# Meowuu7/equi-articulated-pose

Measured on AMD Instinct MI355X. Metric: point-clouds/sec (4096 pts, 60 anchors) fwd+bwd, higher is better.
Workload: dtype f32; 1 GPU; 8 x 4096-pt synthetic laptop clouds per GPU, 3-block inter backbone 1->64->128->512 (NN=64,K=24,A=60), forward+backward+Adam; clouds_per_gpu=8, points=4096, anchors=60

## Files before the change

### equi-articulated-pose_amd/csrc/bn_act.hip

```cpp
#include "common.h"

namespace {

constexpr int TB = 256;
constexpr int VPT = 8;
constexpr int SEG = TB * VPT * 4;

__device__ __forceinline__ float wave_sum(float v) {
#pragma unroll
    for (int o = 32; o > 0; o >>= 1) v += __shfl_xor(v, o);
    return v;
}

__device__ __forceinline__ void block_reduce2(float a, float b, float *pa, float *pb) {
    __shared__ float sa[TB / 64], sb[TB / 64];
    a = wave_sum(a); b = wave_sum(b);
    if ((threadIdx.x & 63) == 0) { sa[threadIdx.x >> 6] = a; sb[threadIdx.x >> 6] = b; }
    __syncthreads();
    if (threadIdx.x == 0) {
        float ta = 0.f, tb = 0.f;
#pragma unroll
        for (int i = 0; i < TB / 64; ++i) { ta += sa[i]; tb += sb[i]; }
        *pa = ta; *pb = tb;
    }
// ... 96 lines not shown
    const size_t o = ((size_t)ci * gridDim.z + bi) * nseg + seg;
    block_reduce2(s, q, pg + o, pgx + o);
}

template <bool CLOUD>
__global__ __launch_bounds__(TB) void bn_act_bwd_apply_kernel(int c, long n, float slope, const float *__restrict__ gy,
                                                             const float *__restrict__ x, const float *__restrict__ scale,
                                                             const float *__restrict__ shift, const float *__restrict__ mean,
                                                             const float *__restrict__ invstd, const float *__restrict__ k2,
                                                             const float *__restrict__ k3, float *__restrict__ gx,
                                                             const float *__restrict__ mask, int na) {
    const int seg = blockIdx.x, ci = blockIdx.y, bi = blockIdx.z;
    const int si = CLOUD ? bi * c + ci : ci;
    const float sc = scale[si], sh = shift[si], mu = mean[si], is = invstd[si], c2 = k2[si], c3 = k3[si];
    const size_t r0 = ((size_t)bi * c + ci) * n;
    const float *mrow = (CLOUD && mask) ? mask + (size_t)bi * (unsigned)(n / na) : nullptr;
    const long base = (long)seg * SEG;
    auto one = [&](float g, float xv, float m) {
        const float pre = fmaf(xv, sc, sh);
        const float gg = pre > 0.f ? g : g * slope;
        if (CLOUD) return fmaf(-m, fmaf((xv - mu) * is, c3, c2), gg * sc);
        return fmaf(gg, sc, -c2) - ((xv - mu) * is) * c3;
    };
#pragma unroll
    for (int v = 0; v < VPT; ++v) {
        const long i = base + ((long)v * TB + threadIdx.x) * 4;
        if (i + 3 < n) {
            const float4 g = *reinterpret_cast<const float4 *>(gy + r0 + i);
            const float4 a = *reinterpret_cast<const float4 *>(x + r0 + i);
            const float m = mrow ? mrow[(unsigned)i / (unsigned)na] : 1.f;
            *reinterpret_cast<float4 *>(gx + r0 + i) = make_float4(one(g.x, a.x, m), one(g.y, a.y, m), one(g.z, a.z, m), one(g.w, a.w, m));
        } else {
            for (long j = i; j < n; ++j) gx[r0 + j] = one(gy[r0 + j], x[r0 + j], mrow ? mrow[(unsigned)j / (unsigned)na] : 1.f);
        }
    }
}

constexpr int RM_PIECES = 16;
__global__ __launch_bounds__(256) void bn_act_bwd_apply_rowmax_kernel(int c, long n4, int nq, float slope, const float4 *__restrict__ gy,
                                                                      const float4 *__restrict__ x, const float *__restrict__ scale,
                                                                      const float *__restrict__ shift, const float *__restrict__ mean,
                                                                      const float *__restrict__ invstd, const float *__restrict__ k2,
                                                                      const float *__restrict__ k3, float4 *__restrict__ gx,
                                                                      unsigned *__restrict__ rowmax) {
    __shared__ unsigned s_max[256][4];
    const int ci = blockIdx.y, bi = blockIdx.z, t = threadIdx.x;
    const int T = nq * (256 / nq);
    const float sc = scale[ci], sh = shift[ci], mu = mean[ci], is = invstd[ci], c2 = k2[ci], c3 = k3[ci];
    const size_t r0 = ((size_t)bi * c + ci) * (size_t)n4;
    const long base = (long)blockIdx.x * RM_PIECES * T;
    auto one = [&](float g, float xv) {
        const float pre = fmaf(xv, sc, sh);
        const float gg = pre > 0.f ? g : g * slope;
        return fmaf(gg, sc, -c2) - ((xv - mu) * is) * c3;
    };
    unsigned m0 = 0, m1 = 0, m2 = 0, m3 = 0;
    if (t < T) {
        float4 g[RM_PIECES], a[RM_PIECES];
#pragma unroll
        for (int v = 0; v < RM_PIECES; ++v) {
            const long i = base + (long)v * T + t;
            if (i < n4) { g[v] = gy[r0 + i]; a[v] = x[r0 + i]; }
        }
#pragma unroll
        for (int v = 0; v < RM_PIECES; ++v) {
            const long i = base + (long)v * T + t;
            if (i < n4) {
                const float4 o = make_float4(one(g[v].x, a[v].x), one(g[v].y, a[v].y), one(g[v].z, a[v].z), one(g[v].w, a[v].w));
                gx[r0 + i] = o;
                m0 = max(m0, __float_as_uint(o.x) & 0x7fffffffu); m1 = max(m1, __float_as_uint(o.y) & 0x7fffffffu);
                m2 = max(m2, __float_as_uint(o.z) & 0x7fffffffu); m3 = max(m3, __float_as_uint(o.w) & 0x7fffffffu);
            }
        }
    }
    s_max[t][0] = m0; s_max[t][1] = m1; s_max[t][2] = m2; s_max[t][3] = m3;
    __syncthreads();
    if (t < 4 * nq) {
        unsigned v = 0;
        for (int u = t >> 2; u < T; u += nq) v = max(v, s_max[u][t & 3]);
        if (v) atomicMax(rowmax + ((size_t)bi * c + ci) * (4 * nq) + t, v);
    }
}

__global__ __launch_bounds__(256) void bn_act_bwd_reduce_fromy_kernel(int c, long n4, int nq, int nblk, float slope, float inv_slope, const float4 *__restrict__ gy,
                                                                      const float4 *__restrict__ y, const float *__restrict__ beta,
                                                                      const float *__restrict__ inv_gamma, float *__restrict__ pg, float *__restrict__ pgx,
                                                                      unsigned *__restrict__ gmax, unsigned *__restrict__ xmax) {
    __shared__ unsigned s_max[256][8];
    const int ci = blockIdx.y, bi = blockIdx.z, t = threadIdx.x;
    const int T = nq * (256 / nq);
    const float be = beta[ci], ig = inv_gamma[ci];
    const size_t r0 = ((size_t)bi * c + ci) * (size_t)n4;
    const long base = (long)blockIdx.x * RM_PIECES * T;
    float s = 0.f, q = 0.f;
    unsigned mg[4] = {0, 0, 0, 0}, mx[4] = {0, 0, 0, 0};
    if (t < T) {
        float4 g[RM_PIECES], a[RM_PIECES];
#pragma unroll
        for (int v = 0; v < RM_PIECES; ++v) {
            const long i = base + (long)v * T + t;
            if (i < n4) { g[v] = gy[r0 + i]; a[v] = y[r0 + i]; }
        }
#pragma unroll
        for (int v = 0; v < RM_PIECES; ++v) {
            const long i = base + (long)v * T + t;
            if (i < n4) {
                const float gv[4] = {g[v].x, g[v].y, g[v].z, g[v].w}, yv[4] = {a[v].x, a[v].y, a[v].z, a[v].w};
#pragma unroll
                for (int e = 0; e < 4; ++e) {
                    const bool pos = yv[e] > 0.f;
                    const float gg = pos ? gv[e] : gv[e] * slope, xh = ((pos ? yv[e] : yv[e] * inv_slope) - be) * ig;
                    s += gg;
                    q = fmaf(gg, xh, q);
                    mg[e] = max(mg[e], __float_as_uint(gg) & 0x7fffffffu);
                    mx[e] = max(mx[e], __float_as_uint(xh) & 0x7fffffffu);
                }
            }
        }
    }
#pragma unroll
    for (int e = 0; e < 4; ++e) { s_max[t][e] = mg[e]; s_max[t][4 + e] = mx[e]; }
    const size_t o = ((size_t)ci * gridDim.z + bi) * nblk + blockIdx.x;
    block_reduce2(s, q, pg + o, pgx + o);
    if (t < 4 * nq) {
        unsigned vg = 0, vx = 0;
        for (int u = t >> 2; u < T; u += nq) { vg = max(vg, s_max[u][t & 3]); vx = max(vx, s_max[u][4 + (t & 3)]); }
        const size_t at = ((size_t)bi * c + ci) * (4 * nq) + t;
        if (vg) atomicMax(gmax + at, vg);
        if (vx) atomicMax(xmax + at, vx);
    }
}

inline int nseg_of(long n) { return (int)((n + SEG - 1) / SEG); }

}

extern "C" int eap_bn_act_segments(int64_t n) { return nseg_of((long)n); }

extern "C" int eap_bn_stats_f32(int b, int c, int64_t n, const float *x, float *psum, float *psq, eap_stream_t stream) {
    if (b <= 0 || c <= 0 || n <= 0) return 0;
    if ((n & 3) != 0) return eap::bad_arg("bn_stats: row length must be a multiple of 4");
    const int nseg = nseg_of(n);
    return eap::run_kernel("bn_stats", bn_stats_kernel<false>, nseg, c, b, dim3(TB), 0, eap::S(stream), c, (long)n, nseg, x, psum, psq, (const float *)nullptr, 1);
}

extern "C" int eap_bn_act_fwd_f32(int b, int c, int64_t n, float slope, const float *x, const float *scale,
                                  const float *shift, float *y, eap_stream_t stream) {
    if (b <= 0 || c <= 0 || n <= 0) return 0;
    if ((n & 3) != 0) return eap::bad_arg("bn_act_fwd: row length must be a multiple of 4");
    return eap::run_kernel("bn_act_fwd", bn_act_fwd_kernel<false, false>, nseg_of(n), c, b, dim3(TB), 0, eap::S(stream), c, (long)n, slope, x, scale, shift,
                           (const float *)nullptr, y);
}

extern "C" int eap_bn_act_add_fwd_f32(int b, int c, int64_t n, float slope, const float *x, const float *scale,
                                      const float *shift, const float *res, float *y, eap_stream_t stream) {
    if (b <= 0 || c <= 0 || n <= 0) return 0;
    if ((n & 3) != 0) return eap::bad_arg("bn_act_add_fwd: row length must be a multiple of 4");
    return eap::run_kernel("bn_act_add_fwd", bn_act_fwd_kernel<true, false>, nseg_of(n), c, b, dim3(TB), 0, eap::S(stream), c, (long)n, slope, x, scale, shift,
                           res, y);
}

extern "C" int eap_bn_act_bwd_reduce_f32(int b, int c, int64_t n, float slope, const float *gy, const float *x,
                                         const float *scale, const float *shift, const float *mean,
                                         const float *invstd, float *pg, float *pgx, eap_stream_t stream) {
    if (b <= 0 || c <= 0 || n <= 0) return 0;
    if ((n & 3) != 0) return eap::bad_arg("bn_act_bwd_reduce: row length must be a multiple of 4");
    const int nseg = nseg_of(n);
    return eap::run_kernel("bn_act_bwd_reduce", bn_act_bwd_reduce_kernel<false>, nseg, c, b, dim3(TB), 0, eap::S(stream), c, (long)n, nseg, slope, gy, x,
                           scale, shift, mean, invstd, pg, pgx);
}

extern "C" int eap_bn_act_bwd_apply_f32(int b, int c, int64_t n, float slope, const float *gy, const float *x,
                                        const float *scale, const float *shift, const float *mean,
                                        const float *invstd, const float *k2, const float *k3, float *gx,
                                        eap_stream_t stream) {
    if (b <= 0 || c <= 0 || n <= 0) return 0;
    if ((n & 3) != 0) return eap::bad_arg("bn_act_bwd_apply: row length must be a multiple of 4");
    return eap::run_kernel("bn_act_bwd_apply", bn_act_bwd_apply_kernel<false>, nseg_of(n), c, b, dim3(TB), 0, eap::S(stream), c, (long)n, slope, gy, x,
                           scale, shift, mean, invstd, k2, k3, gx, (const float *)nullptr, 1);
}

extern "C" int eap_bn_act_bwd_apply_rowmax_f32(int b, int c, int64_t n, int na, float slope, const float *gy, const float *x,
                                               const float *scale, const float *shift, const float *mean,
                                               const float *invstd, const float *k2, const float *k3, float *gx, uint32_t *rowmax,
                                               eap_stream_t stream) {
    if (b <= 0 || c <= 0 || n <= 0) return 0;
    if (na <= 0 || (na & 3) != 0 || na > 256 || n % na != 0 ||
        ((reinterpret_cast<uintptr_t>(gy) | reinterpret_cast<uintptr_t>(x) | reinterpret_cast<uintptr_t>(gx)) & 15) != 0)
        return eap::bad_arg("bn_act_bwd_apply_rowmax: rows of [points][na], na a multiple of 4 up to 256, 16-byte aligned tensors");
    hipStream_t s = eap::S(stream);
    if (int e = eap::hip_fail(hipMemsetAsync(rowmax, 0, sizeof(uint32_t) * (size_t)b * c * na, s), "bn_act_bwd_apply_rowmax memset")) return e;
    const int nq = na / 4, T = nq * (256 / nq);
    const long n4 = (long)(n / 4);
    return eap::run_kernel("bn_act_bwd_apply_rowmax", bn_act_bwd_apply_rowmax_kernel, eap::cdiv(n4, (long)RM_PIECES * T), c, b, dim3(256), 0, s, c, n4, nq,
                           slope, reinterpret_cast<const float4 *>(gy), reinterpret_cast<const float4 *>(x), scale, shift, mean, invstd, k2, k3,
                           reinterpret_cast<float4 *>(gx), rowmax);
}

extern "C" int eap_bn_act_fromy_blocks(int64_t n, int na) {
    if (na <= 0 || (na & 3) != 0 || na > 256) return 0;
    const int nq = na / 4, T = nq * (256 / nq);
    const long n4 = (long)(n / 4);
    return (int)((n4 + (long)RM_PIECES * T - 1) / ((long)RM_PIECES * T));
}

extern "C" int eap_bn_act_bwd_reduce_fromy_f32(int b, int c, int64_t n, int na, float slope, const float *gy, const float *y, const float *beta,
                                               const float *inv_gamma, float *pg, float *pgx, uint32_t *gmax, uint32_t *xmax, eap_stream_t stream) {
    if (b <= 0 || c <= 0 || n <= 0) return 0;
    if (na <= 0 || (na & 3) != 0 || na > 256 || n % na != 0 || !(slope > 0.f) ||
        ((reinterpret_cast<uintptr_t>(gy) | reinterpret_cast<uintptr_t>(y)) & 15) != 0)
        return eap::bad_arg("bn_act_bwd_reduce_fromy: rows of [points][na], na a multiple of 4 up to 256, 16-byte aligned tensors, a positive slope");
    hipStream_t s = eap::S(stream);
    if (int e = eap::hip_fail(hipMemsetAsync(gmax, 0, sizeof(uint32_t) * (size_t)b * c * na, s), "bn_act_bwd_reduce_fromy memset")) return e;
    if (int e = eap::hip_fail(hipMemsetAsync(xmax, 0, sizeof(uint32_t) * (size_t)b * c * na, s), "bn_act_bwd_reduce_fromy memset")) return e;
    const int nq = na / 4, nblk = eap_bn_act_fromy_blocks(n, na);
    return eap::run_kernel("bn_act_bwd_reduce_fromy", bn_act_bwd_reduce_fromy_kernel, nblk, c, b, dim3(256), 0, s, c, (long)(n / 4), nq, nblk, slope,
                           1.0f / slope, reinterpret_cast<const float4 *>(gy), reinterpret_cast<const float4 *>(y), beta, inv_gamma, pg, pgx, gmax, xmax);
}

namespace {
inline int cloud_dims(const char *who, int b, int c, long n, int na, bool masked) {
    char buf[200];
    if ((n & 3) != 0 || n >= (1l << 31)) {
        snprintf(buf, sizeof(buf), "%s: row length must be a multiple of 4 below 2^31", who);
        return eap::bad_arg(buf);
    }
    if (masked && (na <= 0 || (na & 3) != 0 || n % na != 0)) {
        snprintf(buf, sizeof(buf), "%s: with a mask a row is [points][na], na a multiple of 4", who);
        return eap::bad_arg(buf);
    }
    return 0;
}
}

extern "C" int eap_bn_stats_masked_f32(int b, int c, int64_t n, int na, const float *x, const float *mask, float *psum, float *psq,
                                       eap_stream_t stream) {
    if (b <= 0 || c <= 0 || n <= 0) return 0;
    if (!mask) return eap::bad_arg("bn_stats_masked: mask is null");
    if (int e = cloud_dims("bn_stats_masked", b, c, (long)n, na, true)) return e;
    const int nseg = nseg_of(n);
    return eap::run_kernel("bn_stats_masked", bn_stats_kernel<true>, nseg, c, b, dim3(TB), 0, eap::S(stream), c, (long)n, nseg, x, psum, psq, mask, na);
}

extern "C" int eap_bn_act_cloud_fwd_f32(int b, int c, int64_t n, float slope, const float *x, const float *scale, const float *shift,
                                        float *y, eap_stream_t stream) {
    if (b <= 0 || c <= 0 || n <= 0) return 0;
    if (int e = cloud_dims("bn_act_cloud_fwd", b, c, (long)n, 0, false)) return e;
    return eap::run_kernel("bn_act_cloud_fwd", bn_act_fwd_kernel<false, true>, nseg_of(n), c, b, dim3(TB), 0, eap::S(stream), c, (long)n, slope, x, scale,
                           shift, (const float *)nullptr, y);
}

extern "C" int eap_bn_act_cloud_bwd_reduce_f32(int b, int c, int64_t n, float slope, const float *gy, const float *x, const float *scale,
                                               const float *shift, const float *mean, const float *invstd, float *pg, float *pgx,
                                               eap_stream_t stream) {
    if (b <= 0 || c <= 0 || n <= 0) return 0;
    if (int e = cloud_dims("bn_act_cloud_bwd_reduce", b, c, (long)n, 0, false)) return e;
    const int nseg = nseg_of(n);
    return eap::run_kernel("bn_act_cloud_bwd_reduce", bn_act_bwd_reduce_kernel<true>, nseg, c, b, dim3(TB), 0, eap::S(stream), c, (long)n, nseg, slope, gy, x,
                           scale, shift, mean, invstd, pg, pgx);
}

extern "C" int eap_bn_act_cloud_bwd_apply_f32(int b, int c, int64_t n, int na, float slope, const float *gy, const float *x,
                                              const float *scale, const float *shift, const float *mean, const float *invstd,
                                              const float *k2, const float *k3, const float *mask, float *gx, eap_stream_t stream) {
    if (b <= 0 || c <= 0 || n <= 0) return 0;
    if (int e = cloud_dims("bn_act_cloud_bwd_apply", b, c, (long)n, na, mask != nullptr)) return e;
    return eap::run_kernel("bn_act_cloud_bwd_apply", bn_act_bwd_apply_kernel<true>, nseg_of(n), c, b, dim3(TB), 0, eap::S(stream), c, (long)n, slope, gy, x,
                           scale, shift, mean, invstd, k2, k3, gx, mask, mask ? na : 1);
}
```

### equi-articulated-pose_amd/csrc/common.h

```cpp
#pragma once
#include <hip/hip_runtime.h>
#include <stdint.h>
#include <stdio.h>

#include <atomic>

#include "../../include/eap_hip.h"

namespace eap {

void set_error(const char *msg);
void set_kernel(const char *name);

static inline int check_launch(const char *what) {
    hipError_t e = hipGetLastError();
    if (e != hipSuccess) {
        char buf[256];
        snprintf(buf, sizeof(buf), "%s: %s", what, hipGetErrorString(e));
        set_error(buf);
        return (int)e;
    }
    return 0;
}

static inline int bad_arg(const char *what) {
    set_error(what);
    return (int)hipErrorInvalidValue;
}

static inline int hip_fail(hipError_t e, const char *what) {
    if (e == hipSuccess) return 0;
    char buf[256];
    snprintf(buf, sizeof(buf), "%s: %s", what, hipGetErrorString(e));
    set_error(buf);
    return (int)e;
}

static inline hipStream_t S(eap_stream_t s) { return (hipStream_t)s; }

static inline long long cdiv(long long a, long long b) { return (a + b - 1) / b; }

template <typename... P>
static inline bool aligned16(const P *...p) { return ((reinterpret_cast<uintptr_t>(p) | ... | (uintptr_t)0) & 15) == 0; }

static inline int launch_dims(const char *what, long long gx, long long gy, long long gz, dim3 block, dim3 *grid) {
    const bool block_ok = block.x >= 1 && block.y >= 1 && block.z >= 1 && block.x <= 1024 && block.y <= 1024 && block.z <= 1024 &&
                          block.x * block.y * block.z <= 1024;
    if (!block_ok || gx < 1 || gy < 1 || gz < 1 || gx > 0xffffffffLL / block.x || gy > 65535 || gz > 65535) {
        char buf[256];
        snprintf(buf, sizeof(buf), "%s: grid (%lld, %lld, %lld) x block (%u, %u, %u) is outside the launch limits: every size >= 1, block <= 1024 "
                 "threads, grid.x * block.x < 2^32, grid.y and grid.z <= 65535", what, gx, gy, gz, block.x, block.y, block.z);
        return bad_arg(buf);
    }
    *grid = dim3((unsigned)gx, (unsigned)gy, (unsigned)gz);
    return 0;
}

struct LdsOptIn {
    std::atomic<const void *> kernel{nullptr};
    std::atomic<unsigned> bytes[64] = {};
};
inline LdsOptIn g_lds_opt_in[256];

static inline int allow_dynamic_lds(const void *kernel, size_t bytes, const char *what) {
    int dev = 0;
    if (int e = hip_fail(hipGetDevice(&dev), what)) return e;
    std::atomic<unsigned> *seen = nullptr;
    for (size_t i = 0, h = reinterpret_cast<uintptr_t>(kernel) >> 4; i < 256 && dev >= 0 && dev < 64; ++i) {
        LdsOptIn &slot = g_lds_opt_in[(h + i) & 255];
        const void *k = slot.kernel.load(std::memory_order_acquire);
        if (k == nullptr && slot.kernel.compare_exchange_strong(k, kernel, std::memory_order_acq_rel)) k = kernel;
        if (k == kernel) { seen = &slot.bytes[dev]; break; }
    }
    unsigned have = seen ? seen->load(std::memory_order_acquire) : 0u;
    if (have >= bytes) return 0;
    for (;;) {
        if (int e = hip_fail(hipFuncSetAttribute(kernel, hipFuncAttributeMaxDynamicSharedMemorySize, (int)bytes), what)) return e;
        if (!seen || seen->compare_exchange_strong(have, (unsigned)bytes, std::memory_order_acq_rel)) return 0;
        if (have > bytes) bytes = have;
    }
}

template <typename K, typename... Args>
static inline int run_kernel(const char *what, K kernel, long long gx, long long gy, long long gz, dim3 block, size_t lds_bytes, hipStream_t s,
                             Args... args) {
    dim3 grid;
    if (int e = launch_dims(what, gx, gy, gz, block, &grid)) return e;
    if (lds_bytes)
        if (int e = allow_dynamic_lds(reinterpret_cast<const void *>(kernel), lds_bytes, what)) return e;
    hipLaunchKernelGGL(kernel, grid, block, lds_bytes, s, args...);
    return check_launch(what);
}

int side_fork(hipStream_t s, hipStream_t *side);
int side_join(hipStream_t s);
struct SideJoin {
    hipStream_t s;
    bool armed = true;
    explicit SideJoin(hipStream_t stream) : s(stream) {}
    ~SideJoin() { if (armed) side_join(s); }
    int join() { armed = false; return side_join(s); }
};

int reduce_slabs(const float *ws, float *C, long long mn, int N, int slabs, long long ldc, hipStream_t s, const char *what);
bool group_lists_supported(int na, int ks);
int group_lists_fwd(int b, int c, int p, int n, int nn, int na, int ks, float sigma, const float *feats,
                    const int32_t *idx, const float *gx, const float *rk, const int32_t *nonident, int blocked, float *out,
                    hipStream_t s);
int group_lists_inv(int b, int o, int p, int nn, int na, int gy_pitch, int ks, int rcap, float sigma, const float *gy,
                    const int32_t *rows, const int32_t *off, const int32_t *cnt, const int32_t *ent_p,
                    const float *ent_gx, const float *rk, float *z, hipStream_t s);
bool group_lists2_preferred(int c, int na, int ks, int layout);
int group_lists2_fwd(int b, int c, int p, int n, int nn, int na, int ks, float sigma, const float *feats,
                     const int32_t *idx, const float *gx, const float *rk, const int32_t *nonident, int layout, float *out,
                     hipStream_t s);
int group_lists2_inv(int b, int o, int p, int nn, int na, int gy_pitch, int ks, int rcap, float sigma, const float *gy,
                     const int32_t *rows, const int32_t *off, const int32_t *cnt, const int32_t *ent_p,
                     const float *ent_gx, const float *rk, float *z, hipStream_t s);
bool inter_zpconv_rows_supported(int np, int nq, int na, int ks, int nn, int c);
int inter_zpconv_rows_fwd(int b, int np, int nq, int na, int ks, int nn, int c, const int32_t *idx, const float *w,
                          const float *feats, float *out, const int32_t *only_flagged, hipStream_t s);
bool inter_zpconv_mfma_supported(int np, int nq, int na, int ks, int nn, int c);
int inter_zpconv_mfma_fwd(int b, int np, int nq, int na, int ks, int nn, int c, const int32_t *idx0, const float *w,
                          const float *feats, const int32_t *skip, float *out, hipStream_t s);
int zpconv_index_check(int b, int np, int per_point, int nn, const int32_t *idx, int32_t *idx0, float *eid, int32_t *flag, hipStream_t s);
int zpconv_first_rows(int b, int np, int per_point, int nn, const int32_t *idx, int32_t *idx0, hipStream_t s);
// ... 11 lines not shown
```

### equi-articulated-pose_amd/csrc/inv_lists.hip

```cpp
#include "common.h"

namespace {

constexpr int RT = 1024;
constexpr int MAXN = 16384;
constexpr int SORT_COMPACT = 2048;

__global__ __launch_bounds__(256) void inv_count_kernel(int per_cloud, int n, const int32_t *__restrict__ idx,
                                                        int32_t *__restrict__ counts) {
    extern __shared__ int s_hist[];
    const int bi = blockIdx.y, t = threadIdx.x;
    for (int i = t; i < n; i += 256) s_hist[i] = 0;
    __syncthreads();
    const int chunk = (per_cloud + gridDim.x - 1) / gridDim.x;
    const int beg = blockIdx.x * chunk, end = min(per_cloud, beg + chunk);
    const int32_t *src = idx + (size_t)bi * per_cloud;
    for (int e = beg + t; e < end; e += 256) {
        const int q = src[e];
        if ((unsigned)q < (unsigned)n) atomicAdd(&s_hist[q], 1);
    }
    __syncthreads();
    for (int i = t; i < n; i += 256) {
        const int v = s_hist[i];
        if (v) atomicAdd(&counts[(size_t)bi * n + i], v);
// ... 58 lines not shown
            run += (int)c;
        }
    }
    const int total = s_part[RT - 1];
    for (int i = m2 + t; i < n; i += RT) {
        rows[(size_t)bi * n + i] = -1;
        cnt[(size_t)bi * n + i] = 0;
        off[(size_t)bi * n + i] = total;
    }
    if (t == 0) n_rows[bi] = nref;
}

__global__ __launch_bounds__(256) void inv_fill_kernel(int per_cloud, int nn, int n, int rld,
                                                       const int32_t *__restrict__ idx, const float4 *__restrict__ gx,
                                                       const int32_t *__restrict__ rows, const int32_t *__restrict__ off,
                                                       int32_t *__restrict__ ent_p, float4 *__restrict__ ent_gx) {
    __shared__ int s_wave[4];
    const int r = blockIdx.x, bi = blockIdx.y;
    const int q = rows[(size_t)bi * rld + r];
    if (q < 0) return;
    const int t = threadIdx.x, lane = t & 63, wave = t >> 6;
    const int quads = per_cloud >> 2;
    const int qper = (quads + 3) / 4;
    const int qbeg = wave * qper, qend = min(quads, qbeg + qper);
    const int4 *src = reinterpret_cast<const int4 *>(idx + (size_t)bi * per_cloud);
    int mine = 0;
    for (int i = qbeg + lane; i < qend; i += 64) {
        const int4 v = src[i];
        mine += (v.x == q) + (v.y == q) + (v.z == q) + (v.w == q);
    }
    for (int d = 32; d > 0; d >>= 1) mine += __shfl_xor(mine, d);
    if (lane == 0) s_wave[wave] = mine;
    __syncthreads();
    int base = off[(size_t)bi * rld + r];
    for (int w = 0; w < wave; ++w) base += s_wave[w];
    int32_t *dp = ent_p + (size_t)bi * per_cloud;
    float4 *dg = ent_gx + (size_t)bi * per_cloud;
    const float4 *sg = gx + (size_t)bi * per_cloud;
    for (int i0 = qbeg; i0 < qend; i0 += 64) {
        const int i = i0 + lane;
        int4 v = make_int4(-1, -1, -1, -1);
        if (i < qend) v = src[i];
        const bool m0 = v.x == q, m1 = v.y == q, m2 = v.z == q, m3 = v.w == q;
        const unsigned long long b0 = __ballot(m0), b1 = __ballot(m1), b2 = __ballot(m2), b3 = __ballot(m3);
        if ((b0 | b1 | b2 | b3) == 0ull) continue;
        int pos = base;
        pos += __builtin_amdgcn_mbcnt_hi((unsigned)(b0 >> 32), __builtin_amdgcn_mbcnt_lo((unsigned)b0, 0));
        pos += __builtin_amdgcn_mbcnt_hi((unsigned)(b1 >> 32), __builtin_amdgcn_mbcnt_lo((unsigned)b1, 0));
        pos += __builtin_amdgcn_mbcnt_hi((unsigned)(b2 >> 32), __builtin_amdgcn_mbcnt_lo((unsigned)b2, 0));
        pos += __builtin_amdgcn_mbcnt_hi((unsigned)(b3 >> 32), __builtin_amdgcn_mbcnt_lo((unsigned)b3, 0));
        const int e = 4 * i;
        if (m0) { dp[pos] = e / nn; dg[pos] = sg[e]; ++pos; }
        if (m1) { dp[pos] = (e + 1) / nn; dg[pos] = sg[e + 1]; ++pos; }
        if (m2) { dp[pos] = (e + 2) / nn; dg[pos] = sg[e + 2]; ++pos; }
        if (m3) { dp[pos] = (e + 3) / nn; dg[pos] = sg[e + 3]; ++pos; }
        base += __popcll(b0) + __popcll(b1) + __popcll(b2) + __popcll(b3);
    }
}

__global__ __launch_bounds__(256) void rows_gather_kernel(int c, int n, int na4, int rcap, int rld,
                                                          const int32_t *__restrict__ rows, const float4 *__restrict__ src,
                                                          float4 *__restrict__ dst) {
    const int bi = blockIdx.z, ci = blockIdx.y;
    const int e = blockIdx.x * 256 + threadIdx.x;
    if (e >= rcap * na4) return;
    const int r = e / na4, a = e - r * na4;
    const int q = rows[(size_t)bi * rld + r];
    float4 v = make_float4(0.f, 0.f, 0.f, 0.f);
    if (q >= 0) v = src[(((size_t)bi * c + ci) * n + q) * na4 + a];
    dst[(((size_t)bi * c + ci) * rcap + r) * na4 + a] = v;
}

__global__ __launch_bounds__(256) void rows_scatter_kernel(int c, int n, int na4, int rcap, int rld,
                                                           const int32_t *__restrict__ rows, const float4 *__restrict__ src,
                                                           float4 *__restrict__ dst) {
    const int bi = blockIdx.z, ci = blockIdx.y;
    const int e = blockIdx.x * 256 + threadIdx.x;
    if (e >= rcap * na4) return;
    const int r = e / na4, a = e - r * na4;
    const int q = rows[(size_t)bi * rld + r];
    if (q >= 0) dst[(((size_t)bi * c + ci) * n + q) * na4 + a] = src[(((size_t)bi * c + ci) * rcap + r) * na4 + a];
}

}

extern "C" int eap_inv_lists_rows(int b, int p, int n, int nn, const int32_t *idx, int32_t *counts, int32_t *rows,
                                  int32_t *off, int32_t *cnt, int32_t *n_rows, eap_stream_t stream) {
    if (b <= 0 || p <= 0 || nn <= 0 || n <= 0) return 0;
    if (n > MAXN) return eap::bad_arg("inv_lists_rows: more than 16384 support points per cloud");
    if ((long long)p * nn >= (1ll << 31)) return eap::bad_arg("inv_lists_rows: more than 2^31 entries per cloud");
    hipStream_t s = eap::S(stream);
    int e = eap::hip_fail(hipMemsetAsync(counts, 0, sizeof(int32_t) * (size_t)b * n, s), "inv_lists_rows memset");
    if (e) return e;
    const int per_cloud = p * nn;
    e = eap::run_kernel("inv_lists_rows (count)", inv_count_kernel, eap::cdiv(per_cloud, 8192), b, 1, dim3(256), sizeof(int) * n, s, per_cloud, n, idx, counts);
    if (e) return e;
    int n2 = RT;
    while (n2 < n) n2 <<= 1;
    const size_t shmem = sizeof(unsigned long long) * n2;
    return eap::run_kernel("inv_lists_rows (sort)", inv_rows_kernel, b, 1, 1, dim3(RT), shmem, s, n, n2, counts, rows, off, cnt, n_rows);
}

extern "C" int eap_inv_lists_fill(int b, int p, int n, int nn, int rcap, const int32_t *idx, const float *gx,
                                  const int32_t *rows, const int32_t *off, int32_t *ent_p, float *ent_gx,
                                  eap_stream_t stream) {
    if (b <= 0 || p <= 0 || nn <= 0 || rcap <= 0) return 0;
    if (((long long)p * nn & 3) != 0) return eap::bad_arg("inv_lists_fill: p * nn must be a multiple of 4");
    if (rcap > n) return eap::bad_arg("inv_lists_fill: rcap exceeds the number of support points");
    return eap::run_kernel("inv_lists_fill", inv_fill_kernel, rcap, b, 1, dim3(256), 0, eap::S(stream), p * nn, nn, n, n, idx, reinterpret_cast<const float4 *>(gx),
                           rows, off, ent_p, reinterpret_cast<float4 *>(ent_gx));
}

extern "C" int eap_rows_gather_f32(int b, int c, int n, int na, int rcap, int rows_ld, const int32_t *rows,
                                   const float *src, float *dst, eap_stream_t stream) {
    if (b <= 0 || c <= 0 || rcap <= 0) return 0;
    if ((na & 3) != 0) return eap::bad_arg("rows_gather: na must be a multiple of 4");
    return eap::run_kernel("rows_gather", rows_gather_kernel, eap::cdiv((long long)rcap * (na / 4), 256), c, b, dim3(256), 0, eap::S(stream), c, n, na / 4, rcap, rows_ld,
                           rows, reinterpret_cast<const float4 *>(src), reinterpret_cast<float4 *>(dst));
}

extern "C" int eap_rows_scatter_f32(int b, int c, int n, int na, int rcap, int rows_ld, const int32_t *rows,
                                    const float *src, float *dst, eap_stream_t stream) {
    if (b <= 0 || c <= 0) return 0;
    if ((na & 3) != 0) return eap::bad_arg("rows_scatter: na must be a multiple of 4");
    hipStream_t s = eap::S(stream);
    int e = eap::hip_fail(hipMemsetAsync(dst, 0, sizeof(float) * (size_t)b * c * n * na, s), "rows_scatter memset");
    if (e || rcap <= 0) return e;
    return eap::run_kernel("rows_scatter", rows_scatter_kernel, eap::cdiv((long long)rcap * (na / 4), 256), c, b, dim3(256), 0, s, c, n, na / 4, rcap, rows_ld, rows,
                           reinterpret_cast<const float4 *>(src), reinterpret_cast<float4 *>(dst));
}
```

### equi-articulated-pose_amd/csrc/narrow_conv.hip

```cpp
#include "common.h"
#include "device_prims.h"
#include <type_traits>

namespace {

constexpr int NT = 256, WAVES = 4;
constexpr int TILE = 128;
constexpr int SEGC = 2048;

__device__ __forceinline__ int drow(int r, int h) { return (r & 3) + 8 * (r >> 2) + 4 * h; }

template <int KS2>
__device__ __forceinline__ void load_x(f32x4 (&xa)[KS2], const float *__restrict__ xb, long n, long col0, unsigned voff, bool ok, int ck, int h) {
#pragma unroll
    for (int s = 0; s < KS2; ++s)
        xa[s] = (ok && 2 * s + h < ck) ? ld_off<f32x4>(xb + (size_t)(2 * s) * n + col0, voff) : (f32x4){0.f, 0.f, 0.f, 0.f};
}

template <int KS2>
__device__ __forceinline__ void load_w(float (&wf)[KS2], const float *__restrict__ W, int orow, int ck, int h) {
#pragma unroll
    for (int s = 0; s < KS2; ++s) wf[s] = (2 * s + h < ck) ? W[(size_t)orow * ck + 2 * s + h] : 0.f;
}

// ... 57 lines not shown
                                                                 const float *__restrict__ x, float *__restrict__ pivot,
                                                                 float *__restrict__ psum, float *__restrict__ psq) {
    __shared__ __attribute__((aligned(16))) float s_piv[64];
    __shared__ float s_red[WAVES][2][32];
    const Pos w(ct, n);
    const int t = threadIdx.x, o0 = blockIdx.y * ct * 32, h = w.h;
    if (t < 32 * ct) {
        float p = 0.f;
        for (int k = 0; k < ck; ++k) p = fmaf(W[(size_t)(o0 + t) * ck + k], x[(size_t)k * n], p);
        s_piv[t] = p;
        if (w.seg == 0 && w.bi == 0) pivot[o0 + t] = p;
    }
    __syncthreads();
    float wf[KS2];
    load_w<KS2>(wf, W, w.ch0 + w.li, ck, h);
    f32x4 pv[4];
#pragma unroll
    for (int g = 0; g < 4; ++g) pv[g] = *reinterpret_cast<const f32x4 *>(&s_piv[w.ch0 - o0 + 8 * g + 4 * h]);
    float sa[16], qa[16];
#pragma unroll
    for (int r = 0; r < 16; ++r) sa[r] = qa[r] = 0.f;
    const float *xb = x + (size_t)w.bi * ck * n;
#pragma unroll 1
    for (long col0 = w.beg + (long)w.cw * TILE; col0 < w.end; col0 += (long)w.ncw * TILE) {
        const long col = col0 + 4 * w.li;
        const bool ok = col < n;
        f32x4 xa[KS2];
        load_x<KS2>(xa, xb, n, col0, w.xoff, ok, ck, h);
        f32x16 d[4];
        conv_tile<KS2, false>(d, xa, wf);
        if (ok) {
#pragma unroll
            for (int r = 0; r < 16; ++r)
#pragma unroll
                for (int c = 0; c < 4; ++c) {
                    const float dd = d[c][r] - pv[r >> 2][r & 3];
                    sa[r] += dd;
                    qa[r] = fmaf(dd, dd, qa[r]);
                }
        }
    }
    block_sums(sa, qa, s_red, ct, o0, w.bi, gridDim.z, nseg, w.seg, psum, psq);
}

template <int KS2>
__global__ __launch_bounds__(NT) void narrow_conv_bnact_fwd_kernel(int ct, int o, int ck, long n, float slope, const float *__restrict__ W,
                                                                     const float *__restrict__ x, const float *__restrict__ scale,
                                                                     const float *__restrict__ shift, float *__restrict__ y) {
    const Pos w(ct, n);
    const int h = w.h;
    float wf[KS2];
    load_w<KS2>(wf, W, w.ch0 + w.li, ck, h);
    f32x4 sc[4], sh[4];
#pragma unroll
    for (int g = 0; g < 4; ++g) {
        sc[g] = *reinterpret_cast<const f32x4 *>(scale + w.ch0 + 8 * g + 4 * h);
        sh[g] = *reinterpret_cast<const f32x4 *>(shift + w.ch0 + 8 * g + 4 * h);
    }
    const float *xb = x + (size_t)w.bi * ck * n;
    float *yb = y + ((size_t)w.bi * o + w.ch0) * n;
    const unsigned roff = 4u * (4u * h * (unsigned)n + 4u * w.li);
#pragma unroll 1
    for (long col0 = w.beg + (long)w.cw * TILE; col0 < w.end; col0 += (long)w.ncw * TILE) {
        const long col = col0 + 4 * w.li;
        const bool ok = col < n;
        f32x4 xa[KS2];
        load_x<KS2>(xa, xb, n, col0, w.xoff, ok, ck, h);
        f32x16 d[4];
        conv_tile<KS2, false>(d, xa, wf);
        if (ok) {
#pragma unroll
            for (int r = 0; r < 16; ++r) {
                const float a = sc[r >> 2][r & 3], b = sh[r >> 2][r & 3];
                f32x4 v;
                v.x = fmaf(d[0][r], a, b); v.y = fmaf(d[1][r], a, b); v.z = fmaf(d[2][r], a, b); v.w = fmaf(d[3][r], a, b);
                v.x = v.x > 0.f ? v.x : v.x * slope; v.y = v.y > 0.f ? v.y : v.y * slope;
                v.z = v.z > 0.f ? v.z : v.z * slope; v.w = v.w > 0.f ? v.w : v.w * slope;
                st_off<f32x4>(yb + (size_t)(8 * (r >> 2)) * n + col0, roff + 4u * (unsigned)(r & 3) * (unsigned)n, v);
            }
        }
    }
}

template <int KS2>
__global__ __launch_bounds__(NT) void narrow_conv_bwd_reduce_kernel(int ct, int o, int ck, long n, int nseg, float slope,
                                                                      const float *__restrict__ gy, const float *__restrict__ x,
                                                                      const float *__restrict__ W, const float *__restrict__ scale,
                                                                      const float *__restrict__ shift, const float *__restrict__ mean,
                                                                      const float *__restrict__ invstd, float *__restrict__ pg,
                                                                      float *__restrict__ pgx) {
    __shared__ __attribute__((aligned(16))) float s_sc[64], s_sh[64], s_mu[64], s_is[64];
    __shared__ float s_red[WAVES][2][32];
    const Pos w(ct, n);
    const int t = threadIdx.x, o0 = blockIdx.y * ct * 32, h = w.h;
    if (t < 32 * ct) { s_sc[t] = scale[o0 + t]; s_sh[t] = shift[o0 + t]; s_mu[t] = mean[o0 + t]; s_is[t] = invstd[o0 + t]; }
    __syncthreads();
    float wf[KS2];
    load_w<KS2>(wf, W, w.ch0 + w.li, ck, h);
    float sa[16], qa[16];
#pragma unroll
    for (int r = 0; r < 16; ++r) sa[r] = qa[r] = 0.f;
    const float *xb = x + (size_t)w.bi * ck * n;
    const float *gb = gy + ((size_t)w.bi * o + w.ch0) * n;
    const unsigned roff = 4u * (4u * h * (unsigned)n + 4u * w.li);
    const int lc = w.ch0 - o0;
#pragma unroll 1
    for (long col0 = w.beg + (long)w.cw * TILE; col0 < w.end; col0 += (long)w.ncw * TILE) {
        const long col = col0 + 4 * w.li;
        const bool ok = col < n;
        f32x4 xa[KS2];
        load_x<KS2>(xa, xb, n, col0, w.xoff, ok, ck, h);
        f32x16 d[4];
        conv_tile<KS2, false>(d, xa, wf);
        if (ok) {
#pragma unroll
            for (int g = 0; g < 4; ++g) {
                f32x4 gv[4];
#pragma unroll
                for (int q = 0; q < 4; ++q) gv[q] = ld_off<f32x4>(gb + (size_t)(8 * g) * n + col0, roff + 4u * q * (unsigned)n);
                const f32x4 sc = *reinterpret_cast<const f32x4 *>(&s_sc[lc + 8 * g + 4 * h]), sh = *reinterpret_cast<const f32x4 *>(&s_sh[lc + 8 * g + 4 * h]);
                const f32x4 mu = *reinterpret_cast<const f32x4 *>(&s_mu[lc + 8 * g + 4 * h]), is = *reinterpret_cast<const f32x4 *>(&s_is[lc + 8 * g + 4 * h]);
#pragma unroll
                for (int q = 0; q < 4; ++q)
#pragma unroll
                    for (int c = 0; c < 4; ++c) {
                        const float yv = d[c][4 * g + q];
                        const float pre = fmaf(yv, sc[q], sh[q]);
                        const float gg = pre > 0.f ? gv[q][c] : gv[q][c] * slope;
                        sa[4 * g + q] += gg;
                        qa[4 * g + q] = fmaf(gg, (yv - mu[q]) * is[q], qa[4 * g + q]);
                    }
            }
        }
    }
    block_sums(sa, qa, s_red, ct, o0, w.bi, gridDim.z, nseg, w.seg, pg, pgx);
}

template <int KS2>
__global__ __launch_bounds__(NT) void narrow_conv_bwd_dw_kernel(int ct, int o, int ck, long n, int nseg, float slope,
                                                                  const float *__restrict__ gy, const float *__restrict__ x,
                                                                  const float *__restrict__ W, const float *__restrict__ scale,
                                                                  const float *__restrict__ shift, const float *__restrict__ mean,
                                                                  const float *__restrict__ invstd, const float *__restrict__ k2,
                                                                  const float *__restrict__ k3, float *__restrict__ partial) {
    __shared__ float s_part[WAVES][16][64];
    const Pos w(ct, n);
    const int h = w.h, li = w.li, wave = threadIdx.x >> 6;
    const int ch = w.ch0 + li;
    float wf[KS2];
    load_w<KS2>(wf, W, ch, ck, h);
    const float sc = scale[ch], sh = shift[ch], mu = mean[ch], is = invstd[ch], c2 = k2[ch], c3 = k3[ch];
    const float *gb = gy + ((size_t)w.bi * o + w.ch0) * n;
    const unsigned goff = 4u * ((unsigned)li * (unsigned)n + 16u * h), koff = 4u * ((unsigned)min(li, ck - 1) * (unsigned)n + 16u * h);
    f32x16 dw;
#pragma unroll
    for (int r = 0; r < 16; ++r) dw[r] = 0.f;
    const float *xb = x + (size_t)w.bi * ck * n;
    const f32x4 zero4 = {0.f, 0.f, 0.f, 0.f};
#pragma unroll 1
    for (long col0 = w.beg + (long)w.cw * TILE; col0 < w.end; col0 += (long)w.ncw * TILE) {
        const long col = col0 + 4 * li;
        f32x4 xa[KS2];
        load_x<KS2>(xa, xb, n, col0, w.xoff, col < n, ck, h);
        f32x16 d[4];
        conv_tile<KS2, true>(d, xa, wf);
#pragma unroll
        for (int g = 0; g < 4; ++g) {
            f32x4 gv[4], xv[4];
#pragma unroll
            for (int q = 0; q < 4; ++q) {
                const long cq = col0 + 4 * (8 * g + 4 * h + q);
                const bool in = cq < n;
                gv[q] = in ? ld_off<f32x4>(gb + col0 + 4 * (8 * g + q), goff) : zero4;
                xv[q] = (in && li < ck) ? ld_off<f32x4>(xb + col0 + 4 * (8 * g + q), koff) : zero4;
            }
#pragma unroll
            for (int q = 0; q < 4; ++q)
#pragma unroll
                for (int c = 0; c < 4; ++c) {
                    const float yv = d[c][4 * g + q];
                    const float pre = fmaf(yv, sc, sh);
                    const float gg = pre > 0.f ? gv[q][c] : gv[q][c] * slope;
                    const float gx = fmaf(gg, sc, -c2) - ((yv - mu) * is) * c3;
                    dw = __builtin_amdgcn_mfma_f32_32x32x2f32(gx, xv[q][c], dw, 0, 0, 0);
                }
        }
    }
#pragma unroll
    for (int r = 0; r < 16; ++r) s_part[wave][r][w.lane] = dw[r];
    __syncthreads();
    if (wave < ct) {
        float *slab = partial + ((size_t)w.bi * nseg + w.seg) * o * ck;
#pragma unroll
        for (int r = 0; r < 16; ++r) {
            float v = 0.f;
            for (int u = wave; u < WAVES; u += ct) v += s_part[u][r][w.lane];
            if (li < ck) slab[(size_t)(w.ch0 + drow(r, h)) * ck + li] = v;
        }
    }
}

__global__ __launch_bounds__(256) void narrow_conv_dw_sum_kernel(int mn, int slabs, const float *__restrict__ partial, float *__restrict__ dW) {
    const int e = blockIdx.x * 4 + (threadIdx.x >> 6), lane = threadIdx.x & 63;
    if (e >= mn) return;
    float s = 0.f;
    for (int z = lane; z < slabs; z += 64) s += partial[(size_t)z * mn + e];
#pragma unroll
    for (int d = 32; d > 0; d >>= 1) s += __shfl_xor(s, d);
    if (lane == 0) dW[e] = s;
}

inline int nseg_of(long n) { return (int)((n + SEGC - 1) / SEGC); }

inline bool misaligned(const void *p) { return (reinterpret_cast<uintptr_t>(p) & 15) != 0; }

inline int refuse(const char *who, int o, int ck, long n, const void *p0, const void *p1, const void *p2 = nullptr) {
    char buf[200];
    const char *why = nullptr;
    if (ck < 1 || ck > 32) why = "1 to 32 contraction indices (C*K)";
    else if (o < 32 || o % 32 != 0) why = "a multiple of 32 output channels";
    else if (n < 0 || (n & 3) != 0 || n >= (1l << 25)) why = "a row length (P*A) that is a multiple of 4 below 2^25";
    else if (misaligned(p0) || misaligned(p1) || misaligned(p2)) why = "16-byte aligned tensors";
    if (!why) return 0;
    snprintf(buf, sizeof(buf), "%s: takes %s", who, why);
    return eap::bad_arg(buf);
}

inline int tiles_per_block(int o) { return o % 64 == 0 ? 2 : 1; }

template <typename F>
int by_depth(int ck, F &&f) {
    return ck <= 24 ? f(std::integral_constant<int, 12>{}) : f(std::integral_constant<int, 16>{});
}

}

extern "C" int eap_narrow_conv_segments(int64_t n) { return n > 0 ? nseg_of((long)n) : 0; }

extern "C" int eap_narrow_conv_stats_f32(int b, int o, int ck, int64_t n, const float *W, const float *x, float *pivot, float *psum,
                                         float *psq, eap_stream_t stream) {
    if (int e = refuse("narrow_conv_stats", o, ck, (long)n, x, nullptr)) return e;
    if (b <= 0 || n <= 0) return 0;
    const int nseg = nseg_of((long)n), ct = tiles_per_block(o);
    return by_depth(ck, [&](auto ks2) {
        return eap::run_kernel("narrow_conv_stats", narrow_conv_stats_kernel<decltype(ks2)::value>, nseg, o / (32 * ct), b, dim3(NT), 0, eap::S(stream), ct,
                               ck, (long)n, nseg, W, x, pivot, psum, psq);
    });
}

extern "C" int eap_narrow_conv_bnact_fwd_f32(int b, int o, int ck, int64_t n, float slope, const float *W, const float *x, const float *scale,
                                             const float *shift, float *y, eap_stream_t stream) {
    if (int e = refuse("narrow_conv_bnact_fwd", o, ck, (long)n, x, y, scale)) return e;
    if (misaligned(shift)) return eap::bad_arg("narrow_conv_bnact_fwd: takes 16-byte aligned tensors");
    if (b <= 0 || n <= 0) return 0;
    const int ct = tiles_per_block(o);
    return by_depth(ck, [&](auto ks2) {
        return eap::run_kernel("narrow_conv_bnact_fwd", narrow_conv_bnact_fwd_kernel<decltype(ks2)::value>, nseg_of((long)n), o / (32 * ct), b, dim3(NT), 0,
                               eap::S(stream), ct, o, ck, (long)n, slope, W, x, scale, shift, y);
    });
}

extern "C" int eap_narrow_conv_bwd_reduce_f32(int b, int o, int ck, int64_t n, float slope, const float *gy, const float *x, const float *W,
                                              const float *scale, const float *shift, const float *mean, const float *invstd, float *pg,
                                              float *pgx, eap_stream_t stream) {
    if (int e = refuse("narrow_conv_bwd_reduce", o, ck, (long)n, x, gy)) return e;
    if (b <= 0 || n <= 0) return 0;
    const int nseg = nseg_of((long)n), ct = tiles_per_block(o);
    return by_depth(ck, [&](auto ks2) {
        return eap::run_kernel("narrow_conv_bwd_reduce", narrow_conv_bwd_reduce_kernel<decltype(ks2)::value>, nseg, o / (32 * ct), b, dim3(NT), 0, eap::S(stream),
                               ct, o, ck, (long)n, nseg, slope, gy, x, W, scale, shift, mean, invstd, pg, pgx);
    });
}

extern "C" int eap_narrow_conv_bwd_dw_f32(int b, int o, int ck, int64_t n, float slope, const float *gy, const float *x, const float *W,
                                          const float *scale, const float *shift, const float *mean, const float *invstd, const float *k2,
                                          const float *k3, float *partial, float *dW, eap_stream_t stream) {
    if (int e = refuse("narrow_conv_bwd_dw", o, ck, (long)n, x, gy)) return e;
    if (b <= 0 || n <= 0) return 0;
    const int nseg = nseg_of((long)n), ct = tiles_per_block(o);
    hipStream_t s = eap::S(stream);
    int e = by_depth(ck, [&](auto ks2) {
        return eap::run_kernel("narrow_conv_bwd_dw", narrow_conv_bwd_dw_kernel<decltype(ks2)::value>, nseg, o / (32 * ct), b, dim3(NT), 0, s, ct, o, ck, (long)n,
                               nseg, slope, gy, x, W, scale, shift, mean, invstd, k2, k3, partial);
    });
    if (e) return e;
    const int mn = o * ck;
    return eap::run_kernel("narrow_conv_bwd_dw (sum)", narrow_conv_dw_sum_kernel, eap::cdiv(mn, 4), 1, 1, dim3(256), 0, s, mn, b * nseg, partial, dW);
}
```

### equi-articulated-pose_amd/csrc/so3_dense.hip

```cpp
#include <atomic>
#include "common.h"
#include "device_prims.h"
#include <type_traits>

namespace {

typedef unsigned long long u64;
typedef const __attribute__((address_space(4))) unsigned long long *cu64p;

constexpr int KC_BK = 32;
constexpr int KC_LIST_BYTES = 4096;

__host__ __device__ __forceinline__ void dense_kr(int d, int ks, int &k, int &r) {
    const int g = d / (16 * ks), rem = d - g * 16 * ks;
    k = rem >> 4;
    r = 16 * g + (rem & 15);
}


__device__ __forceinline__ void split2(float x0, float x1, unsigned &h, unsigned &l) {
    asm("v_cvt_pk_f16_f32 %0, %2, %3\n\t"
        "v_fma_mixlo_f16 %1, %0, -1.0, %2 op_sel:[0,0,0] op_sel_hi:[1,0,0]\n\t"
        "v_fma_mixhi_f16 %1, %0, -1.0, %3 op_sel:[1,0,0] op_sel_hi:[1,0,0]"
        : "=&v"(h), "=&v"(l) : "v"(x0), "v"(x1));
// ... 174 lines not shown

__global__ __launch_bounds__(256) void dense_rows_kernel(int n_sup, int na, int ks, int rp, int kd_pad, int rows_ld,
                                                         const float *__restrict__ s_xyz, const float *__restrict__ centre,
                                                         const int32_t *__restrict__ rows, const float *__restrict__ rk,
                                                         const float *__restrict__ row_rot, f32x4 *__restrict__ kr) {
    const int b = blockIdx.z, a = blockIdx.y, i = blockIdx.x * 256 + threadIdx.x;
    if (i >= kd_pad) return;
    f32x4 v = {1e4f, 1e4f, 1e4f, 0.f};
    if (i < ks * rp) {
        int k, r;
        dense_kr(i, ks, k, r);
        const int row = rows[(size_t)b * rows_ld + r];
        if ((unsigned)row < (unsigned)n_sup) {
            const float *kp = rk + ((size_t)a * ks + k) * 3;
            double k0 = (double)kp[0], k1 = (double)kp[1], k2 = (double)kp[2];
            if (row_rot != nullptr) {
                const float *M = row_rot + ((size_t)b * rows_ld + r) * 9;
                const double t0 = M[0] * k0 + M[1] * k1 + M[2] * k2, t1 = M[3] * k0 + M[4] * k1 + M[5] * k2, t2 = M[6] * k0 + M[7] * k1 + M[8] * k2;
                k0 = t0; k1 = t1; k2 = t2;
            }
            const double x = (double)s_xyz[((size_t)b * 3 + 0) * n_sup + row] - (double)centre[b * 4 + 0] - k0;
            const double y = (double)s_xyz[((size_t)b * 3 + 1) * n_sup + row] - (double)centre[b * 4 + 1] - k1;
            const double z = (double)s_xyz[((size_t)b * 3 + 2) * n_sup + row] - (double)centre[b * 4 + 2] - k2;
            v = (f32x4){(float)x, (float)y, (float)z, 0.f};
        }
    }
    kr[((size_t)b * na + a) * kd_pad + i] = v;
}

__global__ __launch_bounds__(256) void dense_rowmax_kernel(int m, int l, int na, int seg, long long seg_pitch4, const int32_t *__restrict__ colmap,
                                                           const f32x4 *__restrict__ T, float *__restrict__ scale, float *__restrict__ scale2) {
    __shared__ unsigned s[256][4];
    const int nq = na >> 2, G = 256 / nq, b = blockIdx.y, row = blockIdx.x, t = threadIdx.x;
    const int aq = t % nq, pg = t / nq;
    unsigned v0 = 0, v1 = 0, v2 = 0, v3 = 0;
    if (pg < G) {
        const f32x4 *src = T + ((size_t)b * m + row) * (colmap ? (size_t)1 : (size_t)(l / seg)) * seg_pitch4;
        for (int i0 = pg; i0 < l; i0 += 8 * G) {
            f32x4 q[8];
#pragma unroll
            for (int u = 0; u < 8; ++u) {
                const int i = min(i0 + u * G, l - 1), sg = i / seg;
                if (colmap != nullptr) {
                    const int ci = colmap[(size_t)b * l + i];
                    q[u] = ci >= 0 ? src[(size_t)ci * nq + aq] : (f32x4){0.f, 0.f, 0.f, 0.f};
                } else {
                    q[u] = src[(size_t)sg * seg_pitch4 + (size_t)(i - sg * seg) * nq + aq];
                }
            }
#pragma unroll
            for (int u = 0; u < 8; ++u) {
                v0 = max(v0, __float_as_uint(q[u].x) & 0x7fffffffu);
                v1 = max(v1, __float_as_uint(q[u].y) & 0x7fffffffu);
                v2 = max(v2, __float_as_uint(q[u].z) & 0x7fffffffu);
                v3 = max(v3, __float_as_uint(q[u].w) & 0x7fffffffu);
            }
        }
    }
    s[t][0] = v0; s[t][1] = v1; s[t][2] = v2; s[t][3] = v3;
    __syncthreads();
    if (t < na) {
        unsigned v = 0;
        for (int g = 0; g < G; ++g) v = max(v, s[g * nq + (t >> 2)][t & 3]);
        const float sc = pow2_scale(__uint_as_float(v));
        scale[((size_t)b * na + t) * m + row] = sc;
        scale2[((size_t)b * m + row) * na + t] = sc;
    }
}

__global__ __launch_bounds__(256) void dense_scale_kernel(long long total, int m, int na, const unsigned *__restrict__ rowmax,
                                                          float *__restrict__ scale, float *__restrict__ scale2) {
    const long long i = (long long)blockIdx.x * 256 + threadIdx.x;
    if (i >= total) return;
    const int a = (int)(i % na);
    const long long br = i / na;
    const int row = (int)(br % m);
    const long long b = br / m;
    const float sc = pow2_scale(__uint_as_float(rowmax[i]));
    scale[(b * na + a) * m + row] = sc;
    scale2[i] = sc;
}

struct SplitBn { const f32x4 *Y2; const float *coef; float slope, inv_slope; };
template <bool BN>
__global__ __launch_bounds__(256) __attribute__((amdgpu_waves_per_eu(2, 2))) void dense_split_kernel(int m, int l, int na, int kb_total, int seg, long long seg_pitch4, int mapped,
                                                          const int32_t *__restrict__ n_rows, const int32_t *__restrict__ colmap,
                                                          const f32x4 *__restrict__ T, const float *__restrict__ scale2,
                                                          u32x4 *__restrict__ planes, SplitBn bn) {
    extern __shared__ u32x4 image[];
    const int t = threadIdx.x;
    const int MT = m >> 5;
    const unsigned blk = blockIdx.x >> 1;
    const int kg = (int)(blockIdx.x & 1u), kb = (int)(blk % (unsigned)kb_total), grp_ = (int)(blk / (unsigned)kb_total), mt = grp_ % MT, b = grp_ / MT;
    const int nq = na >> 2, RG = 256 / nq;
    const int aq = t % nq, rr = t / nq;
    const int nseg = l / seg;
    if (mapped && n_rows != nullptr && 16 * kb >= ((min(n_rows[b], seg) + 15) & ~15) * nseg) return;
    const int l0 = 16 * kb + 8 * kg;
    unsigned at[8], keep[8];
    int live = 0;
    if (colmap != nullptr) {
        int ci[8] = {-1, -1, -1, -1, -1, -1, -1, -1};
        if (l0 < l) {
            const int4 c0 = *reinterpret_cast<const int4 *>(colmap + (size_t)b * l + l0), c1 = *reinterpret_cast<const int4 *>(colmap + (size_t)b * l + l0 + 4);
            ci[0] = c0.x; ci[1] = c0.y; ci[2] = c0.z; ci[3] = c0.w; ci[4] = c1.x; ci[5] = c1.y; ci[6] = c1.z; ci[7] = c1.w;
        }
#pragma unroll
        for (int e = 0; e < 8; ++e) { keep[e] = ci[e] >= 0 ? ~0u : 0u; at[e] = (unsigned)max(ci[e], 0) * (unsigned)nq; live |= (int)(keep[e] & 1u) << e; }
    } else {
        int sg = l0 / seg, sr = l0 - sg * seg;
        if (mapped) dense_kr(l0, nseg, sg, sr);
#pragma unroll
        for (int e = 0; e < 8; ++e) {
            keep[e] = l0 + e < l ? ~0u : 0u;
            at[e] = keep[e] ? (unsigned)sg * (unsigned)seg_pitch4 + (unsigned)sr * (unsigned)nq : 0u;
            live |= (int)(keep[e] & 1u) << e;
            if (++sr == seg) { sr = 0; ++sg; }
        }
#pragma unroll
        for (int e = 1; e < 8; ++e) at[e] = keep[e] ? at[e] : at[0];
    }
    if (live == 0)
        for (int i = t; i < 64 * na; i += 256) image[i] = (u32x4){0u, 0u, 0u, 0u};
    for (int it0 = rr; it0 < 32 && rr < RG && live != 0; it0 += 2 * RG) {
        f32x4 q[2][8];
        f32x4 q2[BN ? 2 : 1][BN ? 8 : 1];
        int rowv[2];
#pragma unroll
        for (int u = 0; u < 2; ++u) {
            const int row = 32 * mt + min(it0 + u * RG, 31);
            rowv[u] = row;
            const size_t row_off = ((size_t)b * m + row) * (colmap ? (size_t)1 : (size_t)nseg) * seg_pitch4 + aq;
#pragma unroll
            for (int e = 0; e < 8; ++e) q[u][e] = T[row_off + at[e]];
            if constexpr (BN) {
#pragma unroll
                for (int e = 0; e < 8; ++e) q2[u][e] = bn.Y2[row_off + at[e]];
            }
        }
        __builtin_amdgcn_sched_barrier(0);
        if constexpr (BN) {
#pragma unroll
            for (int u = 0; u < 2; ++u) {
                const float k1 = bn.coef[rowv[u]], k2 = bn.coef[m + rowv[u]], k3 = bn.coef[2 * m + rowv[u]], be = bn.coef[3 * m + rowv[u]], ig = bn.coef[4 * m + rowv[u]];
#pragma unroll
                for (int e = 0; e < 8; ++e)
#pragma unroll
                    for (int j = 0; j < 4; ++j) {
                        const float yv = q2[u][e][j], gv = q[u][e][j];
                        const bool pos = yv > 0.f;
                        const float gg = pos ? gv : gv * bn.slope, pre = pos ? yv : yv * bn.inv_slope;
                        const float gx = fmaf(gg, k1, -k2) - ((pre - be) * ig) * k3;
                        q[u][e][j] = __uint_as_float(__float_as_uint(gx) & keep[e]);
                    }
            }
        } else if (live != 255) {
#pragma unroll
            for (int u = 0; u < 2; ++u)
#pragma unroll
                for (int e = 0; e < 8; ++e)
#pragma unroll
                    for (int j = 0; j < 4; ++j) q[u][e][j] = __uint_as_float(__float_as_uint(q[u][e][j]) & keep[e]);
        }
#pragma unroll
        for (int u = 0; u < 2; ++u) {
            const int i = it0 + u * RG;
            if (i >= 32) break;
            const f32x4 sc = *reinterpret_cast<const f32x4 *>(scale2 + ((size_t)b * m + rowv[u]) * na + 4 * aq);
            u32x4 *dst = image + 256 * aq + ((i + aq) & 31);
#pragma unroll
            for (int j = 0; j < 4; ++j) {
                unsigned h[4], lo[4];
#pragma unroll
                for (int e = 0; e < 4; ++e) split2(q[u][2 * e][j] * sc[j], q[u][2 * e + 1][j] * sc[j], h[e], lo[e]);
                dst[64 * j] = (u32x4){h[0], h[1], h[2], h[3]};
                dst[64 * j + 32] = (u32x4){lo[0], lo[1], lo[2], lo[3]};
            }
        }
    }
    __syncthreads();
    const int w = t >> 6, pl = (t >> 5) & 1, i = t & 31;
    for (int k = 0; k < nq; ++k) {
        const int a = 4 * k + w;
        planes[((((size_t)b * na + a) * kb_total + kb) * MT + mt) * 128 + 64 * pl + 32 * kg + i] = image[64 * a + 32 * pl + ((i + k) & 31)];
    }
}

template <int CSTEPS>
__global__ __launch_bounds__(256) void dense_gplanes_kernel(int m, int na, int ks, int rp, int rch, int kb_total, const float *__restrict__ W3,
                                                            const float *__restrict__ Ft, const int32_t *__restrict__ n_rows,
                                                            const float *__restrict__ bound, float *__restrict__ scale, u32x4 *__restrict__ planes) {
    constexpr int C = 16 * CSTEPS, PITCH = 2 * C + 16;
    extern __shared__ __attribute__((aligned(16))) unsigned char smem[];
    __shared__ unsigned s_red[4];
    const int z = blockIdx.y, b = z / na;
    const int t = threadIdx.x, lane = t & 63, li = lane & 31, kg = lane >> 5, wave = t >> 6;
    const int rows_b = n_rows ? min((min(n_rows[b], rp) + 15) & ~15, rp) : rp;
    unsigned char *Fh = smem, *Fl = smem + (size_t)rch * PITCH;
    const int MT = m >> 5, mt = blockIdx.x * 4 + wave;
    const bool active = mt < MT;
    const int o = 32 * min(mt, MT - 1) + li;
    const float s_out = pow2_scale(bound[(size_t)z * m + o]);
    if (active && kg == 0) scale[(size_t)z * m + o] = s_out;
    for (int rc0 = 0; rc0 < rows_b; rc0 += rch) {
        const int nrows = min(rch, rows_b - rc0);
        if (rc0 > 0) __syncthreads();
        const f32x4 *src = reinterpret_cast<const f32x4 *>(Ft + ((size_t)z * rp + rc0) * C);
        const int n4 = nrows * (C / 4);
        unsigned mx = 0;
        for (int i = t; i < n4; i += 256) {
            const f32x4 v = src[i];
            mx = max(mx, max(max(__float_as_uint(v.x) & 0x7fffffffu, __float_as_uint(v.y) & 0x7fffffffu),
                             max(__float_as_uint(v.z) & 0x7fffffffu, __float_as_uint(v.w) & 0x7fffffffu)));
        }
#pragma unroll
        for (int o_ = 32; o_ > 0; o_ >>= 1) mx = max(mx, (unsigned)__shfl_xor((int)mx, o_));
        if (lane == 0) s_red[wave] = mx;
// ... 489 lines not shown
    const int wtiles = 4 * ((n + 255) / 256), steps = kd / KC_BK;
    return ((int64_t)b * wtiles * steps * 64 + 1) / 2;
}

namespace {
template <int W>
int dense_member(int b, int p, int n_sup, int nn, int rp, int rows_ld, const int32_t *idx, const int32_t *rows, const int32_t *n_rows, int32_t *slot_of,
                 uint32_t *memb, int32_t *flags, eap_stream_t stream) {
    if (b <= 0 || p <= 0) return 0;
    if (rp <= 0 || rp > 32 * W) return eap::bad_arg(W == MEMB_WORDS ? "so3_dense_member: 0 < rp <= 512" : "so3_dense_member_wide: 0 < rp <= 1024");
    hipStream_t s = eap::S(stream);
    if (int e = eap::hip_fail(hipMemsetAsync(slot_of, 0xff, sizeof(int32_t) * (size_t)b * n_sup, s), "so3_dense_member memset")) return e;
    if (int e = eap::hip_fail(hipMemsetAsync(flags, 0, sizeof(int32_t) * (size_t)b, s), "so3_dense_member memset")) return e;
    if (int e = eap::run_kernel("so3_dense_member", dense_slots_kernel, eap::cdiv(rp, 256), b, 1, dim3(256), 0, s, n_sup, rp, rows_ld, rows, n_rows, slot_of)) return e;
    return eap::run_kernel("so3_dense_member", dense_member_kernel<W>, eap::cdiv(p, 256), b, 1, dim3(256), 0, s, p, n_sup, nn, rp, idx, slot_of, memb, flags);
}

template <int W>
int dense_masks(int b, int p, int ks, int rp, int dir, const uint32_t *memb, uint64_t *mask, eap_stream_t stream) {
    if (b <= 0) return 0;
    if (!dense_shape_ok(p, 4, ks, rp, 256, W)) return eap::bad_arg("so3_dense_masks: shape not taken");
    const int n = dir ? p : ks * rp, kd = dir ? ceil_to(ks * rp, KC_BK) : p;
    const int wtiles = 4 * ((n + 255) / 256), steps = kd / KC_BK;
    return eap::run_kernel("so3_dense_masks", dense_mask_kernel<W>, eap::cdiv((long long)wtiles * steps, 4), b, 1, dim3(256), 0, eap::S(stream), p, ks, rp, dir, wtiles, steps,
                           memb, reinterpret_cast<unsigned *>(mask));
}
}

extern "C" int eap_so3_dense_member(int b, int p, int n_sup, int nn, int rp, int rows_ld, const int32_t *idx, const int32_t *rows,
                                    const int32_t *n_rows, int32_t *slot_of, uint32_t *memb, int32_t *flags, eap_stream_t stream) {
    return dense_member<MEMB_WORDS>(b, p, n_sup, nn, rp, rows_ld, idx, rows, n_rows, slot_of, memb, flags, stream);
}

extern "C" int eap_so3_dense_member_wide(int b, int p, int n_sup, int nn, int rp, int rows_ld, const int32_t *idx, const int32_t *rows,
                                         const int32_t *n_rows, int32_t *slot_of, uint32_t *memb, int32_t *flags, eap_stream_t stream) {
    return dense_member<MEMB_WORDS_WIDE>(b, p, n_sup, nn, rp, rows_ld, idx, rows, n_rows, slot_of, memb, flags, stream);
}

extern "C" int eap_so3_dense_masks(int b, int p, int ks, int rp, int dir, const uint32_t *memb, uint64_t *mask, eap_stream_t stream) {
    return dense_masks<MEMB_WORDS>(b, p, ks, rp, dir, memb, mask, stream);
}

extern "C" int eap_so3_dense_masks_wide(int b, int p, int ks, int rp, int dir, const uint32_t *memb, uint64_t *mask, eap_stream_t stream) {
    return dense_masks<MEMB_WORDS_WIDE>(b, p, ks, rp, dir, memb, mask, stream);
}

extern "C" int eap_so3_dense_tables_f32(int b, int p, int n_sup, int na, int ks, int rp, int rows_ld, float sigma, const float *q_xyz,
                                        const float *s_xyz, const int32_t *rows, const float *rk, const float *row_rot, float *centre, float *pt,
                                        float *kr, eap_stream_t stream) {
    if (b <= 0) return 0;
    if (!(sigma > 0.f)) return eap::bad_arg("so3_dense_tables: sigma > 0");
    hipStream_t s = eap::S(stream);
    const int p_pad = ceil_to(p, KC_BK), kd_pad = ceil_to(ks * rp, KC_BK);
    if (int e = eap::run_kernel("so3_dense_tables", dense_centre_kernel, b, 1, 1, dim3(256), 0, s, n_sup, s_xyz, centre)) return e;
    if (int e = eap::run_kernel("so3_dense_tables", dense_points_kernel, eap::cdiv(p_pad, 256), b, 1, dim3(256), 0, s, p, p_pad, q_xyz, centre,
                                reinterpret_cast<f32x4 *>(pt)))
        return e;
    return eap::run_kernel("so3_dense_tables", dense_rows_kernel, eap::cdiv(kd_pad, 256), na, b, dim3(256), 0, s, n_sup, na, ks, rp, kd_pad, rows_ld,
                           s_xyz, centre, rows, rk, row_rot, reinterpret_cast<f32x4 *>(kr));
}

extern "C" int eap_so3_dense_split_f32(int b, int m, int l, int na, int seg, int64_t seg_pitch, int mapped, const int32_t *n_rows, const uint32_t *rowmax,
                                       const int32_t *colmap, const float *src, float *scale, void *planes, eap_stream_t stream) {
    if (b <= 0) return 0;
    if (colmap != nullptr) {
        if (mapped || seg_pitch <= 0 || (l & 7) != 0 || (reinterpret_cast<uintptr_t>(colmap) & 15) != 0)
            return eap::bad_arg("so3_dense_split: a column map (16-byte aligned, a multiple of 8 columns) comes with the source row pitch and without the dense-index mapping");
        seg = l;
    }
    if (seg <= 0) { seg = l; seg_pitch = (int64_t)l * na; }
    if ((m % 32) != 0 || (na % 4) != 0 || na > 64 || (reinterpret_cast<uintptr_t>(src) & 15) || l % seg != 0 ||
        (seg_pitch & 3) != 0 || (colmap == nullptr && seg_pitch < (int64_t)seg * na) || (mapped && ((seg % 16) != 0 || ((l / seg) % 2) != 0)))
        return eap::bad_arg("so3_dense_split: m % 32, na % 4, na <= 64, 16-byte aligned source, whole segments of a 16-byte aligned pitch (mapped: seg % 16, an even number of segments)");
    if ((colmap ? (int64_t)1 : (int64_t)(l / seg)) * (seg_pitch / 4) > 0x7fffffffLL) return eap::bad_arg("so3_dense_split: a source row of at most 2^31 16-byte pieces");
    hipStream_t s = eap::S(stream);
    const int kb_total = ceil_to(l, KC_BK) / 16;
    float *scale2 = scale + (size_t)b * na * m;
    const int e = rowmax != nullptr
                      ? eap::run_kernel("so3_dense_split", dense_scale_kernel, eap::cdiv((long long)b * m * na, 256), 1, 1, dim3(256), 0, s, (long long)b * m * na, m, na, rowmax, scale, scale2)
                      : eap::run_kernel("so3_dense_split", dense_rowmax_kernel, m, b, 1, dim3(256), 0, s, m, l, na, seg, (long long)(seg_pitch / 4), colmap,
                                        reinterpret_cast<const f32x4 *>(src), scale, scale2);
    if (e) return e;
    return eap::run_kernel("so3_dense_split", dense_split_kernel<false>, (long long)kb_total * (m / 32) * b * 2, 1, 1, dim3(256), (size_t)na * 1024, s, m, l, na, kb_total, seg, (long long)(seg_pitch / 4),
                           mapped ? 1 : 0, n_rows, colmap, reinterpret_cast<const f32x4 *>(src), scale2, reinterpret_cast<u32x4 *>(planes), SplitBn{nullptr, nullptr, 1.f, 1.f});
}

extern "C" int eap_so3_dense_split_bn_f32(int b, int m, int l, int l_src, int na, const uint32_t *rowbound, const int32_t *colmap, const float *grad,
                                          const float *act, const float *coef, float slope, float *scale, void *planes, eap_stream_t stream) {
    if (b <= 0) return 0;
    if (colmap == nullptr && l != l_src) return eap::bad_arg("so3_dense_split_bn: without a column map l = l_src");
    if ((m % 32) != 0 || (na % 4) != 0 || na > 64 || ((reinterpret_cast<uintptr_t>(grad) | reinterpret_cast<uintptr_t>(act)) & 15) ||
        (colmap != nullptr && ((l & 7) != 0 || (reinterpret_cast<uintptr_t>(colmap) & 15) != 0)) || rowbound == nullptr || coef == nullptr || !(slope > 0.f))
        return eap::bad_arg("so3_dense_split_bn: m % 32, na % 4, na <= 64, 16-byte aligned sources, a bound per row, a positive slope (column map: 16-byte aligned, l % 8)");
    if ((int64_t)l_src * na / 4 > 0x7fffffffLL) return eap::bad_arg("so3_dense_split_bn: a source row of at most 2^31 16-byte pieces");
    hipStream_t s = eap::S(stream);
    const int kb_total = ceil_to(l, KC_BK) / 16;
    float *scale2 = scale + (size_t)b * na * m;
    if (int e = eap::run_kernel("so3_dense_split_bn", dense_scale_kernel, eap::cdiv((long long)b * m * na, 256), 1, 1, dim3(256), 0, s, (long long)b * m * na, m, na, rowbound, scale,
                                scale2))
        return e;
    const int seg = colmap ? l : l_src;
    return eap::run_kernel("so3_dense_split_bn", dense_split_kernel<true>, (long long)kb_total * (m / 32) * b * 2, 1, 1, dim3(256), (size_t)na * 1024, s, m, l, na, kb_total, seg,
                           (long long)l_src * na / 4, 0, nullptr, colmap, reinterpret_cast<const f32x4 *>(grad), scale2, reinterpret_cast<u32x4 *>(planes),
                           SplitBn{reinterpret_cast<const f32x4 *>(act), coef, slope, 1.0f / slope});
}

namespace {
int untranspose_args(const char *what, int o, int p, int na, const float *yt, const float *y) {
    char buf[256];
    const char *why = nullptr;
    if (o <= 0 || p <= 0) why = "o > 0 and p > 0";
    else if (na <= 0 || (na % 4) != 0) why = "na % 4 == 0 (rows of Y are stored as 16-byte pieces)";
    else if (na > 64) why = "na <= 64 (the tile of a block)";
    else if (yt == nullptr || (reinterpret_cast<uintptr_t>(yt) & 15) != 0) why = "yt 16-byte aligned";
    else if (y == nullptr || (reinterpret_cast<uintptr_t>(y) & 15) != 0) why = "y 16-byte aligned";
    if (why == nullptr) return 0;
    snprintf(buf, sizeof(buf), "%s: %s", what, why);
    return eap::bad_arg(buf);
}

int untranspose_tile(const char *what, int b, int o, int p, int na, int p_dst, const int32_t *map, const float *yt, float *y, const float *bn_scale,
                     const float *bn_shift, float slope, eap_stream_t stream) {
    return eap::run_kernel(what, dense_untranspose_tile_kernel, (long long)eap::cdiv(p, UT_PTS) * o * b, 1, 1, dim3(256), sizeof(float) * (size_t)na * UT_PTS,
                           eap::S(stream), o, p, na, p_dst, map, yt, y, bn_scale, bn_shift, slope);
}
}

extern "C" int eap_so3_dense_untranspose_bnact_f32(int b, int o, int p, int na, int p_dst, const int32_t *map, const float *yt, const float *bn_scale,
                                                   const float *bn_shift, float slope, float *y, eap_stream_t stream) {
    if (b <= 0) return 0;
    if (bn_scale == nullptr || bn_shift == nullptr || (map != nullptr && p_dst <= 0) || (map == nullptr && p_dst != p))
        return eap::bad_arg("so3_dense_untranspose_bnact: scale and shift per channel; p_dst = p without a map");
    if (int e = untranspose_args("so3_dense_untranspose_bnact", o, p, na, yt, y)) return e;
    return untranspose_tile("so3_dense_untranspose_bnact", b, o, p, na, p_dst, map, yt, y, bn_scale, bn_shift, slope, stream);
}

extern "C" int eap_so3_dense_gplanes_supported(int o, int c, int na, int ks, int rp) {
    return (o % 32) == 0 && (c == 64 || c == 128) && na > 0 && ks > 0 && (ks % 2) == 0 && rp > 0 && (rp % 16) == 0;
}

extern "C" int eap_so3_dense_gplanes_f32(int b, int o, int c, int na, int ks, int rp, const float *W3, const float *Ft, const int32_t *n_rows,
                                         const float *bound, float *scale, void *planes, eap_stream_t stream) {
    if (b <= 0) return 0;
    if (!eap_so3_dense_gplanes_supported(o, c, na, ks, rp) ||
        ((reinterpret_cast<uintptr_t>(W3) | reinterpret_cast<uintptr_t>(Ft) | reinterpret_cast<uintptr_t>(planes)) & 15) != 0)
        return eap::bad_arg("so3_dense_gplanes: shape not taken (eap_so3_dense_gplanes_supported), 16-byte aligned operands");
    const int kb_total = ceil_to(ks * rp, KC_BK) / 16;
    const int fit = (int)((84u * 1024u) / ((size_t)(2 * c + 16) * 2)) / 16 * 16;
    const int rch = min(rp, max(fit, 32));
    const size_t shmem = (size_t)rch * (2 * c + 16) * 2;
    return eap::run_kernel("so3_dense_gplanes", c == 128 ? dense_gplanes_kernel<8> : dense_gplanes_kernel<4>, eap::cdiv(o / 32, 4), (long long)b * na, 1, dim3(256), shmem,
                           eap::S(stream), o, na, ks, rp, rch, kb_total, W3, Ft, n_rows, bound, scale, reinterpret_cast<u32x4 *>(planes));
}

extern "C" int eap_so3_dense_product_steps_f32(int dir, int b, int o, int p, int na, int ks, int rp, int64_t ldz, float sigma, const int32_t *n_rows,
                                               const void *planes, const float *scale, const float *pt, const float *kr, const uint64_t *mask,
                                               const int32_t *steps, float *out, eap_stream_t stream) {
    if (b <= 0) return 0;
    if (!eap_so3_dense_supported(p, na, ks, rp, o)) return eap::bad_arg("so3_dense_product: shape not taken (eap_so3_dense_supported)");
    const int p_pad = ceil_to(p, KC_BK), kd_pad = ceil_to(ks * rp, KC_BK);
    KcArgs g;
    g.MT = o / 32; g.na = na; g.zcount = b * na; g.row_slots = rp;
    g.N = dir ? p : ks * rp;
    g.KS = (dir ? kd_pad : p) / KC_BK;
    const bool wide = (o % 256) == 0;
    g.tiles_m = wide ? o / 256 : o / 128;
    g.blocks_n = (g.N + 255) / 256;
    g.mask_tiles = 4 * g.blocks_n;
    g.A = reinterpret_cast<const u32x4 *>(planes);
    g.scale = scale;
    const f32x4 *ptT = reinterpret_cast<const f32x4 *>(pt), *krT = reinterpret_cast<const f32x4 *>(kr);
    if (dir == 0) {
        g.strT = ptT; g.strB = p_pad; g.strA = 0;
        g.colT = krT; g.colB = (long long)na * kd_pad; g.colA = kd_pad;
        if (ldz < (int64_t)na * rp) return eap::bad_arg("so3_dense_product: ldz < na rp");
        g.cB = (long long)o * ks * ldz; g.cA = rp; g.ldm = (long long)ks * ldz; g.rp = rp; g.kstride = ldz;
    } else {
        g.strT = krT; g.strB = (long long)na * kd_pad; g.strA = kd_pad;
        g.colT = ptT; g.colB = p_pad; g.colA = 0;
        g.cB = (long long)na * o * p; g.cA = (long long)o * p; g.ldm = p; g.rp = p; g.kstride = 0;
    }
    g.mask = reinterpret_cast<const unsigned *>(mask);
    g.steps = (steps != nullptr && g.KS <= KC_LIST_BYTES / 4) ? steps : nullptr;
    g.C = out;
    g.neg_inv_sigma = -1.0f / sigma;
    g.n_rows = n_rows; g.ks = ks; g.trim = dir ? 2 : 1;
    if (n_rows == nullptr) g.trim = dir ? 0 : 3;
// ... 78 lines not shown
```

### equi-articulated-pose_amd/vgtk/_hip.py

```python
import ctypes
import os
import re
import struct
import types
import weakref

import torch

_PKG_ROOT = os.path.abspath(os.path.join(os.path.dirname(__file__), '..'))
LIB_PATH = os.path.join(_PKG_ROOT, 'libeap_hip.so')

if not os.path.exists(LIB_PATH):
    raise ImportError(
        f'{LIB_PATH} not found: build the HIP extension first '
        '(python -c "import __graft_entry__ as g; g.build()" or make -C equi-articulated-pose_amd/csrc). '
        'This package has no CPU fallback.')

lib = ctypes.CDLL(LIB_PATH)


_HEADERS = (os.path.join(_PKG_ROOT, 'include', 'eap_hip.h'), os.path.join(os.path.dirname(_PKG_ROOT), 'include', 'eap_hip.h'))
HEADER_PATH = next((p for p in _HEADERS if os.path.exists(p)), _HEADERS[-1])

_I64 = ctypes.c_int64
# ... 973 lines not shown
    b, o, p, na = gy.shape
    ldz = na * geo.rp if ldz is None else int(ldz)
    colmap = geo.columns(None)
    l = p if colmap is None else colmap.shape[1]
    scale = torch.empty(2, b, na, o, dtype=torch.float32, device=gy.device)
    planes = torch.empty(b * na * o * ((l + 31) // 32 * 32), dtype=torch.int32, device=gy.device)
    call('eap_so3_dense_split_bn_f32', gy, b, o, l, p, na, rowbound.view(torch.int32), colmap, gy, yact, coef, slope, scale, planes)
    z = torch.empty(b, o, geo.ks, ldz, dtype=torch.float32, device=gy.device)
    return _dense_product(0, geo, b, o, l, ldz, scale, planes, z, 2.0 * b * o * l * na * geo.ks * geo.nn)


def _partials(x, b, c, n):
    nseg = int(abi.eap_bn_act_segments(n))
    return (torch.empty(c, b * nseg, dtype=torch.float32, device=x.device),
            torch.empty(c, b * nseg, dtype=torch.float32, device=x.device))


_STATS_HINT = [None]
STATS_HINTS_TAKEN = 0


def _leave_hint(slot, t, payload):
    slot[0] = (weakref.ref(t), t._version, tuple(t.shape), payload)


def _take_hint(slot, t):
    h, slot[0] = slot[0], None
    if not USE_ROWMAX_HINT or h is None or h[0]() is not t or h[1] != t._version or h[2] != tuple(t.shape):
        return None
    return h[3]


def leave_stats_hint(t, partials):
    _leave_hint(_STATS_HINT, t, partials)


def take_stats_hint(t):
    global STATS_HINTS_TAKEN
    partials = _take_hint(_STATS_HINT, t)
    STATS_HINTS_TAKEN += partials is not None
    return partials


def bn_stats(x, b, c, n):
    hint = take_stats_hint(x)
    if hint is not None and hint[0].shape[0] == c:
        return hint[0].sum(1, dtype=torch.float64), hint[1].sum(1, dtype=torch.float64)
    ps, pq = _partials(x, b, c, n)
    call('eap_bn_stats_f32', x, b, c, n, x, ps, pq)
    return ps.sum(1, dtype=torch.float64), pq.sum(1, dtype=torch.float64)


def bn_act_fwd(x, b, c, n, scale, shift, slope, residual=None):
    y = torch.empty_like(x)
    if residual is None:
        call('eap_bn_act_fwd_f32', x, b, c, n, slope, x, scale, shift, y)
    else:
        call('eap_bn_act_add_fwd_f32', x, b, c, n, slope, x, scale, shift, residual, y)
    return y


def bn_act_bwd_reduce(gy, x, b, c, n, scale, shift, mean, invstd, slope):
    pg, pgx = _partials(x, b, c, n)
    call('eap_bn_act_bwd_reduce_f32', x, b, c, n, slope, gy, x, scale, shift, mean, invstd, pg, pgx)
    return pg.sum(1, dtype=torch.float64), pgx.sum(1, dtype=torch.float64)


_ROWMAX_HINT = [None]
USE_ROWMAX_HINT = True
ROWMAX_HINTS_TAKEN = 0


def leave_rowmax_hint(t, rowmax):
    _leave_hint(_ROWMAX_HINT, t, rowmax)


def take_rowmax_hint(t):
    global ROWMAX_HINTS_TAKEN
    rowmax = _take_hint(_ROWMAX_HINT, t)
    ROWMAX_HINTS_TAKEN += rowmax is not None
    return rowmax


def bn_act_bwd_apply(gy, x, b, c, n, scale, shift, mean, invstd, k2, k3, slope):
    gx = torch.empty_like(x)
    if x.dim() == 4 and x.shape[3] % 4 == 0 and x.shape[3] <= 64 and n == x.shape[2] * x.shape[3] and c % 128 == 0 and gx.data_ptr() % 16 == 0 \
            and gy.data_ptr() % 16 == 0 and x.data_ptr() % 16 == 0:
        rowmax = torch.empty(b, c, x.shape[3], dtype=torch.int32, device=x.device)
        call('eap_bn_act_bwd_apply_rowmax_f32', x, b, c, n, int(x.shape[3]), slope, gy, x, scale, shift, mean, invstd, k2, k3, gx, rowmax)
        leave_rowmax_hint(gx, rowmax)
        return gx
    call('eap_bn_act_bwd_apply_f32', x, b, c, n, slope, gy, x, scale, shift, mean, invstd, k2, k3, gx)
    return gx



NARROW_CONV_MAX_CK = 32


def narrow_conv_takes(o, ck, n):
    return 1 <= ck <= NARROW_CONV_MAX_CK and o >= 32 and o % 32 == 0 and n % 4 == 0 and n < (1 << 25)


def _narrow_partials(x, b, o, n):
    nseg = int(abi.eap_narrow_conv_segments(n))
    return (torch.empty(o, b * nseg, dtype=torch.float32, device=x.device),
            torch.empty(o, b * nseg, dtype=torch.float32, device=x.device))


def narrow_conv_stats(W, x, partials=False):
    check_input(W, x)
    b, ck, n = x.shape
    o = W.shape[0]
    ps, pq = _narrow_partials(x, b, o, n)
    pivot = torch.empty(o, dtype=torch.float32, device=x.device)
    call('eap_narrow_conv_stats_f32', x, b, o, ck, n, W, x, pivot, ps, pq)
    if partials:
        return ps, pq, pivot
    return ps.sum(1, dtype=torch.float64), pq.sum(1, dtype=torch.float64), pivot.double()


def narrow_conv_bnact_fwd(W, x, scale, shift, slope):
    check_input(W, x, scale, shift)
    b, ck, n = x.shape
    o = W.shape[0]
    y = torch.empty(b, o, n, dtype=torch.float32, device=x.device)
    call('eap_narrow_conv_bnact_fwd_f32', x, b, o, ck, n, slope, W, x, scale, shift, y)
    return y


def narrow_conv_bwd_reduce(gy, x, W, scale, shift, mean, invstd, slope, partials=False):
    check_input(gy, x, W, scale, shift, mean, invstd)
    b, ck, n = x.shape
    o = W.shape[0]
    pg, pgx = _narrow_partials(x, b, o, n)
    call('eap_narrow_conv_bwd_reduce_f32', x, b, o, ck, n, slope, gy, x, W, scale, shift, mean, invstd, pg, pgx)
    if partials:
        return pg, pgx
    return pg.sum(1, dtype=torch.float64), pgx.sum(1, dtype=torch.float64)


def narrow_conv_bwd_dw(gy, x, W, scale, shift, mean, invstd, k2, k3, slope):
    check_input(gy, x, W, scale, shift, mean, invstd, k2, k3)
    b, ck, n = x.shape
    o = W.shape[0]
    nseg = int(abi.eap_narrow_conv_segments(n))
    partial = torch.empty(b * nseg, o, ck, dtype=torch.float32, device=x.device)
    dW = torch.empty(o, ck, dtype=torch.float32, device=x.device)
    call('eap_narrow_conv_bwd_dw_f32', x, b, o, ck, n, slope, gy, x, W, scale, shift, mean, invstd, k2, k3, partial, dW)
    return dW



def bn_stats_masked(x, b, c, n, na, mask):
    ps, pq = _partials(x, b, c, n)
    call('eap_bn_stats_masked_f32', x, b, c, n, na, x, mask, ps, pq)
    return ps.view(c, b, -1).sum(2, dtype=torch.float64).t(), pq.view(c, b, -1).sum(2, dtype=torch.float64).t()


def bn_act_cloud_fwd(x, b, c, n, scale, shift, slope):
    y = torch.empty_like(x)
    call('eap_bn_act_cloud_fwd_f32', x, b, c, n, slope, x, scale, shift, y)
    return y


def bn_act_cloud_bwd_reduce(gy, x, b, c, n, scale, shift, mean, invstd, slope):
    pg, pgx = _partials(x, b, c, n)
    call('eap_bn_act_cloud_bwd_reduce_f32', x, b, c, n, slope, gy, x, scale, shift, mean, invstd, pg, pgx)
    return pg.view(c, b, -1).sum(2, dtype=torch.float64).t(), pgx.view(c, b, -1).sum(2, dtype=torch.float64).t()


def bn_act_cloud_bwd_apply(gy, x, b, c, n, na, scale, shift, mean, invstd, k2, k3, mask, slope):
    gx = torch.empty_like(x)
    call('eap_bn_act_cloud_bwd_apply_f32', x, b, c, n, na, slope, gy, x, scale, shift, mean, invstd, k2, k3, mask, gx)
    return gx



def bn_act_cloud_mean_fwd(x, scale, shift, w, inv_den, slope):
    b, c, p, na = x.shape
    out = torch.empty(b, c, na, dtype=torch.float32, device=x.device)
    call('eap_bn_act_cloud_mean_fwd_f32', x, b, c, p, na, slope, x, scale, shift, w, inv_den, out)
    return out


def bn_act_cloud_mean_bwd_reduce(g, x, scale, shift, mean, invstd, w, inv_den, slope):
    b, c, p, na = x.shape
    parts = int(abi.eap_bn_act_cloud_mean_parts(p))
    pg = torch.empty(b, c, parts, dtype=torch.float32, device=x.device)
    pgx = torch.empty_like(pg)
    call('eap_bn_act_cloud_mean_bwd_reduce_f32', x, b, c, p, na, slope, g, x, scale, shift, mean, invstd, w, inv_den, pg, pgx)
    return pg.sum(2, dtype=torch.float64), pgx.sum(2, dtype=torch.float64)


def bn_act_cloud_mean_bwd_apply(g, x, scale, shift, mean, invstd, k2, k3, w, inv_den, stat_mask, slope):
    b, c, p, na = x.shape
    gx = torch.empty_like(x)
    call('eap_bn_act_cloud_mean_bwd_apply_f32', x, b, c, p, na, slope, g, x, scale, shift, mean, invstd, k2, k3, w, inv_den, stat_mask, gx)
    return gx



def bn_act_cloud_mean_wide_fwd(x, scale, shift, w, inv_den, slope):
    b, c, p, na = x.shape
    out = torch.empty(b, c, na, dtype=torch.float32, device=x.device)
    call('eap_bn_act_cloud_mean_wide_fwd_f32', x, b, c, p, na, slope, x, scale, shift, w, inv_den, out)
    return out


def bn_act_cloud_mean_wide_bwd_reduce(g, x, scale, shift, mean, invstd, w, inv_den, slope):
    b, c, p, na = x.shape
    parts = int(abi.eap_bn_act_cloud_mean_wide_parts(p))
    pg = torch.empty(b, c, parts, dtype=torch.float32, device=x.device)
    pgx = torch.empty_like(pg)
    call('eap_bn_act_cloud_mean_wide_bwd_reduce_f32', x, b, c, p, na, slope, g, x, scale, shift, mean, invstd, w, inv_den, pg, pgx)
    return pg.sum(2, dtype=torch.float64), pgx.sum(2, dtype=torch.float64)


def bn_act_cloud_mean_wide_bwd_apply(g, x, scale, shift, mean, invstd, k2, k3, w, inv_den, stat_mask, slope):
    b, c, p, na = x.shape
    gx = torch.empty_like(x)
    call('eap_bn_act_cloud_mean_wide_bwd_apply_f32', x, b, c, p, na, slope, g, x, scale, shift, mean, invstd, k2, k3, w, inv_den, stat_mask, gx)
    return gx



def _slot_f32(*tensors):
    check_input(*tensors)
    for t in tensors:
        if t is not None and t.dtype != torch.float32:
            raise RuntimeError(f'slot attention kernels take float32 tensors, not {t.dtype}')


# ... 75 lines not shown
```

### equi-articulated-pose_amd/vgtk/so3conv/functional.py

```python
import math
import os
import weakref

import numpy as np
import torch

import vgtk
import vgtk.functional as fr
import vgtk.pc as pctk
import vgtk.spconv as zpconv
import vgtk.cuda.grouping as cuda_nn

from .. import _hip
from . import norm_fold

inter_so3conv_feat_grouping = zpconv.inter_zpconv_grouping_naive
batched_index_select = zpconv.batched_index_select
batched_index_select_other = zpconv.batched_index_select_other

MATERIALIZE_INTER_W = False

GAMMA_SIZE = 3
ROOT = vgtk.__path__[0]
Rs, R_idx, canonical_relative = fr.icosahedron_so3(GAMMA_SIZE)
# ... 832 lines not shown
        b1 = min(b, b0 + step)
        x = _hip.so3_inter_group_fwd(feats[b0:b1], idx[b0:b1], gx[b0:b1], rk, mult, sigma,
                                     None if nonident is None else nonident[b0:b1], blocked=layout, coset=coset, store_order=tp)
        _contract_into(Wc, x, y[b0:b1].view(b1 - b0, o, p * na), layout, folded, b0,
                       x_bound=None if x_bound is None else (x_bound[b0:b1], na, 1.0))
        x = x if keep else None
    return y, x


def _forward_map(feats, W, args, keep, folded):
    idx, gx, rk, amap = args.idx, args.gx, args.rk, args.amap
    b, na = feats.shape[0], feats.shape[3]
    p, o = idx.shape[1], W.shape[0]
    y = torch.empty(b, o, p, na, dtype=torch.float32, device=feats.device)
    step = max(1, b if keep else X_CHUNK_CLOUDS)
    x = None
    for b0 in range(0, b, step):
        b1 = min(b, b0 + step)
        x = _hip.so3_inter_group_fwd_map(feats[b0:b1], idx[b0:b1], gx[b0:b1], rk, amap[b0:b1], args.sigma)
        _contract_into(W, x, y[b0:b1].view(b1 - b0, o, p * na), 0, folded, b0)
        x = x if keep else None
    return y, x


def _forward_res(feats, W, args, keep, folded):
    idx, gx, rk, shift = args.idx, args.gx, args.rk, args.shift
    b, na4 = feats.shape[0], feats.shape[3]
    p, o = idx.shape[1], W.shape[0]
    y = torch.empty(b, o, p, na4, dtype=torch.float32, device=feats.device)
    step = max(1, b if keep else X_CHUNK_CLOUDS)
    x = None
    for b0 in range(0, b, step):
        b1 = min(b, b0 + step)
        x = _hip.so3_inter_group_fwd_res(feats[b0:b1], idx[b0:b1], gx[b0:b1], rk, shift[b0:b1], args.sigma)
        _contract_into(W, x, y[b0:b1].view(b1 - b0, o, p * na4), 0, folded, b0)
        x = x if keep else None
    return y, x


def _backward_res(gy, W, feats, x, args, need_f, need_w):
    b, c, n, na4 = feats.shape
    idx, gx, rk, shift = args.idx, args.gx, args.rk, args.shift
    p, ks = idx.shape[1], rk.shape[1]
    o, ck, pa = W.shape[0], c * ks, p * na4
    gF = gW = None
    if need_w:
        if x is None:
            x = _hip.so3_inter_group_fwd_res(feats, idx, gx, rk, shift, args.sigma)
        gW = torch.empty_like(W)
        _hip.matmul_reduce(gy.view(b, o, pa), x.view(b, ck, pa).transpose(1, 2), gW)
        x = None
    if need_f:
        gx_ = torch.empty(b, ck, pa, dtype=torch.float32, device=gy.device)
        Wt = W.t().contiguous()
        _hip.matmul(Wt, gy.view(b, o, pa), gx_)
        gF = _hip.so3_inter_group_bwd_res(gx_.view(b, c, ks, p, na4), idx, gx, rk, shift, args.sigma, n)
    return gF, gW



def _forward_narrow(feats, W, args, train_ep):
    idx, rk = args.idx, args.rk
    b, c, _, na = feats.shape
    p, ks, o = idx.shape[1], rk.shape[1], W.shape[0]
    x = _hip.so3_inter_group_fwd(feats, idx, args.gx, rk, args.mult, args.sigma, args.nonident).view(b, c * ks, p * na)
    if train_ep.takes_partials(x):
        scale, shift, slope = train_ep.moments_from_partials(*_hip.narrow_conv_stats(W, x, partials=True), b * p * na)
    else:
        s1, s2, pivot = _hip.narrow_conv_stats(W, x)
        scale, shift, slope = train_ep.moments(s1, s2, pivot, b * p * na)
    y = _hip.narrow_conv_bnact_fwd(W, x, scale, shift, slope).view(b, o, p, na)
    train_ep.applied = True
    mean, invstd = train_ep.stats
    return y, x, (scale, shift, mean.float(), invstd.float(), train_ep.saved[3], slope, bool(train_ep.norm.sync))


def _native_norm_bwd(gy, count, sync):
    return bool(_hip.NATIVE_NORM_GLUE and gy.is_cuda and isinstance(count, int) and not norm_fold._syncing(sync))


def _backward_narrow(gy, W, x, bn, need_w):
    scale, shift, mean, invstd, count, slope, sync = bn
    b, o = gy.shape[0], gy.shape[1]
    gy = gy.view(b, o, -1)
    if _native_norm_bwd(gy, count, sync):
        g_bn_w, g_bn_b, k2, k3 = _hip.norm_fold_bwd(*_hip.narrow_conv_bwd_reduce(gy, x, W, scale, shift, mean, invstd, slope, partials=True), scale, count)
        return (_hip.narrow_conv_bwd_dw(gy, x, W, scale, shift, mean, invstd, k2, k3, slope) if need_w else None), g_bn_w, g_bn_b
    sg, sgx = _hip.narrow_conv_bwd_reduce(gy, x, W, scale, shift, mean, invstd, slope)
    gW = None
    if need_w:
        k2, k3 = norm_fold.backward_coefficients(scale, sg, sgx, count, True, sync)
        gW = _hip.narrow_conv_bwd_dw(gy, x, W, scale, shift, mean, invstd, k2, k3, slope)
    return gW, sgx.float(), sg.float()



def _weight_operand(W, c, ks, pad_c=None):
    o = W.shape[0]
    W2 = W.view(o, c, ks).permute(1, 0, 2).reshape(c, o * ks).contiguous()
    if pad_c is not None and pad_c != c:
        W2 = torch.cat([W2, torch.zeros(pad_c - c, o * ks, dtype=torch.float32, device=W.device)])
    return W2


def _rows_grad_from_z(z, W2, c, rp, na, ldz, anchor_major, z_bound=None, reorder=None):
    b, (pad_c, oks) = z.shape[0], W2.shape
    gFc = torch.empty(b, pad_c, ldz, dtype=torch.float32, device=z.device)
    _hip.matmul(W2, z.view(b, oks, ldz), gFc, b_bound=z_bound)
    if anchor_major:
        return gFc[:, :c, :rp * na].reshape(b, c, na, rp).transpose(2, 3)
    gFc = gFc.view(b, c, rp, na)
    return gFc if reorder is None else _hip.anchor_reorder(gFc, reorder)


def _weight_grad_rows(z, fc4, o, ks, ldz, anchor_major, reorder=None):
    b, c, rp, na = fc4.shape
    if reorder is not None:
        fc4 = _hip.anchor_reorder(fc4, reorder)
    fc = fc4.transpose(2, 3).contiguous() if anchor_major else fc4
    return _weight_grad_from_z(z, fc.view(b, c, rp * na), b, c, o, ks, rp * na, ldz)



def _backward_dense(gy, W, feats, head, geo, bn, yact, need_f, need_w):
    b, c, n, na = feats.shape
    o, ks, p, rp = W.shape[0], geo.ks, gy.shape[2], geo.rp
    if BACKWARD_LOG is not None:
        BACKWARD_LOG.append({'channels': (c, o), 'support_rows': n, 'referenced_rows_max': int(rp), 'regime': 'dense rows',
                             **({'norm': 'in the node'} if bn is not None else {})})
    ra = na * rp
    pad_c = 128 if (c == 64 and bn is not None) else c
    ldz = _hip.dense_pitch(ra) if (pad_c % 128 == 0 and (o * ks) % 16 == 0 and need_f) else ra
    gF = gW = g_bn_w = g_bn_b = z_bound = None
    if bn is not None:
        k1, beta, inv_gamma, count, slope, sync = bn
        native = _native_norm_bwd(gy, count, sync)
        if native:
            pg, pgx, gmax, xmax = _hip.bn_act_bwd_reduce_fromy(gy, yact, beta, inv_gamma, slope, partials=True)
            g_bn_w, g_bn_b, _, _, coef, bound, colmax = _hip.norm_fold_bwd(pg, pgx, k1, count, beta, inv_gamma, gmax, xmax)
        else:
            sg, sgx, gmax, xmax = _hip.bn_act_bwd_reduce_fromy(gy, yact, beta, inv_gamma, slope)
            g_bn_w, g_bn_b = sgx.float(), sg.float()
            k2, k3 = norm_fold.backward_coefficients(k1, sg, sgx, count, True, sync)
            coef = torch.stack([k1, k2, k3, beta, inv_gamma]).contiguous()
            bound = (k1.abs()[None, :, None] * gmax + k2.abs()[None, :, None] + k3.abs()[None, :, None] * xmax).contiguous()
        z = _hip.so3_dense_bwd_bn(gy, yact, geo, ldz, coef, bound, slope)
        if ldz % 4 == 0 and rp % 4 == 0 and native:
            z_bound = (_hip.so3_dense_zbound(colmax, head.cnt, head.n_rows, rp, p, ldz).view(torch.int32), 4, 1.0)
        elif ldz % 4 == 0 and rp % 4 == 0:
            live = torch.arange(rp, device=gy.device)[None, :] < head.n_rows[:, None]
            cntf = torch.where(live, head.cnt[:, :rp], torch.zeros_like(head.cnt[:, :rp])).clamp(min=0, max=p).to(torch.float32)
            cols = bound.amax(1)[:, :, None] * cntf[:, None, :]
            words = torch.zeros(b, ldz // 4, dtype=torch.float32, device=gy.device)
            words[:, :ra // 4] = cols.view(b, na, rp // 4, 4).amax(3).view(b, ra // 4)
            z_bound = (words.view(torch.int32), 4, 1.0)
    else:
        z = _hip.so3_dense_bwd(gy, geo, ldz)
    if need_f:
        gFr = _rows_grad_from_z(z, _weight_operand(W, c, ks, pad_c), c, rp, na, ldz, True, z_bound)
        gF = _hip.rows_scatter(gFr.contiguous(), head.rows, n)
    if need_w:
        gW = _weight_grad_rows(z, _hip.rows_gather(feats, head.rows, rp), o, ks, ldz, True)
    return gF, gW, g_bn_w, g_bn_b


def _backward_dense_parts(gy, W, feats, head, pd, need_f, need_w):
    b, c, n, na = feats.shape
    o, ks, rp = W.shape[0], pd.ks, pd.rp
    ra = na * rp
    if BACKWARD_LOG is not None:
        BACKWARD_LOG.append({'channels': (c, o), 'support_rows': n, 'referenced_rows_max': int(rp), 'regime': 'dense rows', 'parts': pd.parts.n})
    ldz = _hip.dense_pitch(ra) if (c % 128 == 0 and (o * ks) % 16 == 0 and need_f) else ra
    W2 = _weight_operand(W, c, ks) if need_f else None
    fc0 = _hip.rows_gather(feats, head.rows, rp) if need_w else None
    gFr = gW = None
    rowmax = _hip.take_rowmax_hint(gy)
    for i, geo in enumerate(pd.geo):
        perm = pd.perm[i]
        z = _hip.so3_dense_bwd(gy, geo, ldz, colmap=pd.parts.col_map[i], rowmax=rowmax)
        pe = None if perm is None else perm[:, None].expand(b, c, rp, na)
        if need_f:
            t = _rows_grad_from_z(z, W2, c, rp, na, ldz, True)
            if gFr is None:
                gFr = torch.zeros(b, c, rp, na, dtype=torch.float32, device=gy.device)
            if pe is None:
                gFr += t
            else:
                gFr.scatter_add_(3, pe, t.contiguous())
        if need_w:
            gw = _weight_grad_rows(z, fc0 if pe is None else fc0.gather(3, pe), o, ks, ldz, True)
            gW = gw if gW is None else gW + gw
        del z
    gF = _hip.rows_scatter(gFr, head.rows, n) if need_f else None
    return gF, gW


def _backward_lists(gy, W, feats, idx, gx, rk, mult, args, head, rcap, any_nonident, need_f, need_w):
    b, c, n, na = feats.shape
    p, ks, o = idx.shape[1], rk.shape[1], W.shape[0]
    gF = gW = None
    rcap = min((rcap + 3) & ~3, n)
    head.wait()
    rows = head.rows[:, :rcap].contiguous()
    off, cnt = head.off[:, :rcap].contiguous(), head.cnt[:, :rcap].contiguous()
    ent_p, ent_gx = head.entries if head.entries is not None else _hip.inv_lists_fill(idx, gx, head.rows, head.off, rcap)
    multinv = _group_tables_inverse(mult) if (mult is not None and any_nonident) else None
    coset = _coset_tables(multinv, args.ident) if multinv is not None else None
    z_order = z_pos = None
    if coset is not None and _hip.so3_group_perm_lists2_takes(o, na, ks, p):
        z_order, z_pos = coset[0], coset[2]
        ent_pc, ent_gx2 = _hip.so3_perm_entries(ent_p, ent_gx, coset[1], args.anchors, args.ident, na, p)
        z = _hip.so3_inter_group_inv_perm2(_hip.anchor_reorder(gy, z_order), rows, off, cnt, ent_pc, ent_gx2, rk, z_order,
                                           args.sigma, idx.shape[2])
    else:
        z = _hip.so3_inter_group_inv(gy, rows, off, cnt, ent_p, ent_gx, rk, multinv, args.sigma, idx.shape[2],
                                     args.ident, args.anchors, coset)
    if need_f:
        gFr = _rows_grad_from_z(z, _weight_operand(W, c, ks), c, rcap, na, rcap * na, False, reorder=z_pos)
        gF = _hip.rows_scatter(gFr, rows, n)
    if need_w:
        gW = _weight_grad_rows(z, _hip.rows_gather(feats, rows, rcap), o, ks, rcap * na, False, reorder=z_order)
    return gF, gW


def _backward_textbook(gy, W, feats, x, idx, gx, rk, mult, nonident, args, layout, need_f, need_w):
    b, c, n, na = feats.shape
    p, ks = idx.shape[1], rk.shape[1]
    o, ck, pa = W.shape[0], c * ks, p * na
    gF = gW = None
    if x is None:
        x = _hip.so3_inter_group_fwd(feats, idx, gx, rk, mult, args.sigma, nonident, blocked=layout,
                                     coset=_coset_tables(mult, args.ident) if (mult is not None and layout == 2) else None)
    if need_w:
        gW = torch.empty_like(W)
        if layout == 2:
            _hip.matmul_reduce(gy.view(b, o, pa), x.view(b, pa, ck), gW)
        elif layout == 1:
            _hip.gemm_reduce(0, 1, o, ck, pa, gy, pa, o * pa, x, pa, ck * pa, gW, ck, b, b_blocked=True)
        else:
            _hip.matmul_reduce(gy.view(b, o, pa), x.view(b, ck, pa).transpose(1, 2), gW)
    if need_f:
        gx_ = torch.empty_like(x.view(b, ck, pa))
        Wt = W.t().contiguous()
# ... 614 lines not shown
```

### include/eap_hip.h

```cpp
#ifndef EAP_HIP_H
#define EAP_HIP_H

#include <stdint.h>

#ifdef __cplusplus
extern "C" {
#endif

typedef void *eap_stream_t;

const char *eap_last_error(void);
int eap_launch_dims_ok(int64_t gx, int64_t gy, int64_t gz, int bx, int by, int bz);
const char *eap_last_kernel(void);
int eap_abi_version(void);


int eap_ball_query_f32(int b, int n, int m, float radius, int nsample, const float *new_xyz,
                       const float *xyz, int32_t *idx, eap_stream_t stream);
int eap_ball_query_f64(int b, int n, int m, float radius, int nsample, const double *new_xyz,
                       const double *xyz, int32_t *idx, eap_stream_t stream);

int eap_furthest_point_sampling_f32(int b, int n, int m, const float *xyz, float *temp,
                                    int32_t *idx, eap_stream_t stream);
int eap_furthest_point_sampling_f64(int b, int n, int m, const double *xyz, double *temp,
// ... 85 lines not shown
                                     eap_stream_t stream);

int eap_so3_inter_group_bwd_f32(int b, int c, int p, int n, int nn, int na, int ks, float sigma,
                                const float *gout, const int32_t *idx, const float *gx,
                                const float *rk, const uint8_t *mult, float *gfeats,
                                eap_stream_t stream);

int64_t eap_so3_inter_group_bwd_workspace(int b, int c, int p, int n, int na);
int eap_so3_inter_group_bwd_slab_f32(int b, int c, int p, int n, int nn, int na, int ks, float sigma,
                                     const float *gout, const int32_t *idx, const float *gx,
                                     const float *rk, const uint8_t *mult, int identity_anchor,
                                     float *gfeats, float *workspace, eap_stream_t stream);


int eap_so3_anchor_map_f32(int b, int p, int n, int nn, int na, const int32_t *idx, const float *q_pose,
                           const float *s_pose, const float *anchors, uint8_t *amap, int32_t *nontrivial,
                           eap_stream_t stream);

int eap_so3_inter_group_fwd_map_f32(int b, int c, int p, int n, int nn, int na, int ks, float sigma,
                                    const float *feats, const int32_t *idx, const float *gx, const float *rk,
                                    const uint8_t *amap, float *out, eap_stream_t stream);

int64_t eap_so3_inter_group_bwd_map_workspace(int b, int c, int p, int n, int na);
int eap_so3_inter_group_bwd_map_f32(int b, int c, int p, int n, int nn, int na, int ks, float sigma,
                                    const float *gout, const int32_t *idx, const float *gx, const float *rk,
                                    const uint8_t *amap, float *gfeats, float *workspace, eap_stream_t stream);


int eap_so3_residual_index_f32(int b, int p, int n, int nn, const int32_t *idx, const float *q_pose,
                               const float *s_pose, const float *res, uint8_t *shift, int32_t *nontrivial,
                               eap_stream_t stream);

int eap_so3_inter_group_fwd_res_f32(int b, int c, int p, int n, int nn, int na, int ks, float sigma,
                                    const float *feats, const int32_t *idx, const float *gx, const float *rk,
                                    const uint8_t *shift, float *out, eap_stream_t stream);

int64_t eap_so3_inter_group_bwd_res_workspace(int b, int c, int p, int n, int na);
int eap_so3_inter_group_bwd_res_f32(int b, int c, int p, int n, int nn, int na, int ks, float sigma,
                                    const float *gout, const int32_t *idx, const float *gx, const float *rk,
                                    const uint8_t *shift, float *gfeats, float *workspace, eap_stream_t stream);

int eap_so3_group_lists_tiles(int tiles);
int eap_so3_group_lists_store16(int on);
int eap_so3_group_perm_lists2(int on);
int eap_so3_group_perm_lists2_takes(int channels, int na, int ks, int n_support);
int eap_so3_perm_entries_f32(int b, int per_cloud, int na, int n_support, const int32_t *ent_p, const float *ent_gx, const uint8_t *code,
                             const float *anchors, int identity_anchor, const int32_t *nonident, int32_t *ent_pc, float *ent_gx2,
                             eap_stream_t stream);
int eap_so3_inter_group_fwd_perm2_t_f32(int b, int c, int p, int n, int nn, int na, int ks, float sigma, const float *feats,
                                        const float *feats_c, const int32_t *idx, const float *gx, const int32_t *ent_pc,
                                        const float *ent_gx2, const float *rk, const uint8_t *order, const int32_t *nonident,
                                        int store_order_columns, float *out, eap_stream_t stream);
int eap_so3_group_fwd_tp_takes(int c, int na, int ks);
int eap_so3_group_fwd_tp_columns(int c, int ks, int32_t *perm);
int eap_so3_inter_group_fwd_tp_f32(int b, int c, int p, int n, int nn, int na, int ks, float sigma, const float *feats,
                                   const int32_t *idx, const float *gx, const float *rk, float *out, eap_stream_t stream);
int eap_so3_inter_group_inv_perm2_f32(int b, int o, int p, int nn, int na, int ks, int rcap, float sigma, const float *gy,
                                      const int32_t *rows, const int32_t *off, const int32_t *cnt, const int32_t *ent_pc,
                                      const float *ent_gx2, const float *rk, const uint8_t *order, float *z, eap_stream_t stream);

int eap_so3_inter_group_inv_f32(int b, int o, int p, int nn, int na, int ks, int rcap, float sigma,
                                const float *gy, const int32_t *rows, const int32_t *off,
                                const int32_t *cnt, const int32_t *ent_p, const float *ent_gx,
                                const float *rk, const uint8_t *multinv, const float *anchors,
                                int identity_anchor, float *z, eap_stream_t stream);
int eap_anchor_reorder_f32(int64_t rows, int na, const float *src, const uint8_t *order, float *dst, eap_stream_t stream);
int eap_anchor_reorder_clouds_f32(int b, int64_t rows_per_cloud, int na, const float *src, const uint8_t *order,
                                  const int32_t *nonident, float *dst, eap_stream_t stream);
int eap_so3_inter_group_inv_coset_f32(int b, int o, int p, int nn, int na, int ks, int rcap, float sigma,
                                      const float *gy, const int32_t *rows, const int32_t *off, const int32_t *cnt,
                                      const int32_t *ent_p, const float *ent_gx, const float *rk, const uint8_t *multinv,
                                      const float *anchors, int identity_anchor, const uint8_t *coset_order,
                                      const uint8_t *coset_code, float *z, eap_stream_t stream);

int eap_inv_lists_rows(int b, int p, int n, int nn, const int32_t *idx, int32_t *counts, int32_t *rows,
                       int32_t *off, int32_t *cnt, int32_t *n_rows, eap_stream_t stream);
int eap_inv_lists_fill(int b, int p, int n, int nn, int rcap, const int32_t *idx, const float *gx,
                       const int32_t *rows, const int32_t *off, int32_t *ent_p, float *ent_gx,
                       eap_stream_t stream);
int eap_rows_gather_f32(int b, int c, int n, int na, int rcap, int rows_ld, const int32_t *rows,
                        const float *src, float *dst, eap_stream_t stream);
int eap_rows_scatter_f32(int b, int c, int n, int na, int rcap, int rows_ld, const int32_t *rows,
                         const float *src, float *dst, eap_stream_t stream);

int eap_so3_dense_supported(int p, int na, int ks, int rp, int o);
int eap_so3_dense_member(int b, int p, int n, int nn, int rp, int rows_ld, const int32_t *idx, const int32_t *rows,
                         const int32_t *n_rows, int32_t *slot_of, uint32_t *memb, int32_t *flags, eap_stream_t stream);
int64_t eap_so3_dense_mask_words(int b, int p, int ks, int rp, int dir);
int eap_so3_dense_masks(int b, int p, int ks, int rp, int dir, const uint32_t *memb, uint64_t *mask, eap_stream_t stream);
int eap_so3_dense_tables_f32(int b, int p, int n, int na, int ks, int rp, int rows_ld, float sigma, const float *q_xyz,
                             const float *s_xyz, const int32_t *rows, const float *rk, const float *row_rot, float *centre, float *pt,
                             float *kr, eap_stream_t stream);
int eap_so3_dense_split_f32(int b, int m, int l, int na, int seg, int64_t seg_pitch, int mapped, const int32_t *n_rows, const uint32_t *rowmax,
                            const int32_t *colmap, const float *src, float *scale, void *planes, eap_stream_t stream);
int eap_so3_dense_product_f32(int dir, int b, int o, int p, int na, int ks, int rp, int64_t ldz, float sigma, const int32_t *n_rows, const void *planes,
                              const float *scale,
                              const float *pt, const float *kr, const uint64_t *mask, float *out, eap_stream_t stream);
int eap_so3_dense_untranspose_f32(int b, int o, int p, int na, const float *yt, float *y, float *psum, float *psq, eap_stream_t stream);
int eap_so3_dense_untranspose_map_f32(int b, int o, int p, int na, int p_dst, const int32_t *map, const float *yt, float *y,
                                      eap_stream_t stream);
int eap_so3_dense_untranspose_map_stats_f32(int b, int o, int p, int na, int p_dst, const int32_t *map, const int32_t *pivot_pos, const float *yt,
                                            float *y, float *psum, float *psq, eap_stream_t stream);
int eap_so3_dense_split_bn_f32(int b, int m, int l, int l_src, int na, const uint32_t *rowbound, const int32_t *colmap, const float *grad,
                               const float *act, const float *coef, float slope, float *scale, void *planes, eap_stream_t stream);
int eap_so3_dense_untranspose_bnact_f32(int b, int o, int p, int na, int p_dst, const int32_t *map, const float *yt, const float *bn_scale,
                                        const float *bn_shift, float slope, float *y, eap_stream_t stream);
int eap_so3_dense_gplanes_supported(int o, int c, int na, int ks, int rp);
int eap_so3_dense_gplanes_f32(int b, int o, int c, int na, int ks, int rp, const float *W3, const float *Ft, const int32_t *n_rows,
                              const float *bound, float *scale, void *planes, eap_stream_t stream);
int eap_so3_dense_point_keys(int b, int p, const uint32_t *memb, int32_t *keys, eap_stream_t stream);
int64_t eap_so3_dense_steps_words(int b, int p, int ks, int rp, int dir);
int eap_so3_dense_steps(int b, int p, int ks, int rp, int dir, int skip, const int32_t *n_rows, const uint64_t *mask, int32_t *steps,
                        eap_stream_t stream);
int eap_so3_dense_product_steps_f32(int dir, int b, int o, int p, int na, int ks, int rp, int64_t ldz, float sigma, const int32_t *n_rows,
                                    const void *planes, const float *scale, const float *pt, const float *kr, const uint64_t *mask,
                                    const int32_t *steps, float *out, eap_stream_t stream);
int eap_so3_dense_max_rows(void);
int eap_so3_dense_member_wide(int b, int p, int n, int nn, int rp, int rows_ld, const int32_t *idx, const int32_t *rows,
                              const int32_t *n_rows, int32_t *slot_of, uint32_t *memb, int32_t *flags, eap_stream_t stream);
int eap_so3_dense_point_keys_wide(int b, int p, const uint32_t *memb, int64_t *keys, eap_stream_t stream);
int eap_so3_dense_masks_wide(int b, int p, int ks, int rp, int dir, const uint32_t *memb, uint64_t *mask, eap_stream_t stream);
int eap_so3_dense_steps_wide(int b, int p, int ks, int rp, int dir, int skip, const int32_t *n_rows, const uint64_t *mask, int32_t *steps,
                             eap_stream_t stream);
int64_t eap_so3_dense_probe_workspace(int b);
int eap_so3_dense_probe(int b, int p, int words, const int32_t *n_rows, const int32_t *nonident, const int32_t *dflags,
                        const uint32_t *memb, const float *rot_a, int64_t blocks_a, const float *rot_b, int64_t blocks_b,
                        const float *rot_cloud, const float *norm_w, const float *norm_b, int channels, float ratio,
                        int32_t *work, int32_t *out, eap_stream_t stream);


int eap_so3_intra_group_fwd_f32(int b, int c, int p, int na, int t, const float *feats,
                                const int32_t *intra_idx, float *out, eap_stream_t stream);
int eap_so3_intra_group_bwd_f32(int b, int c, int p, int na, int t, const float *gout,
                                const int32_t *intra_idx, float *gfeats, eap_stream_t stream);



int eap_gemm_f32(int transA, int transB, int M, int N, int K, const float *A, int64_t lda,
                 int64_t strideA, const float *B, int64_t ldb, int64_t strideB, float *C,
                 int64_t ldc, int64_t strideC, int batch, eap_stream_t stream);

int64_t eap_gemm_f32_reduce_workspace(int M, int N, int K, int batch);
int eap_gemm_f32_reduce(int transA, int transB, int M, int N, int K, const float *A, int64_t lda,
                        int64_t strideA, const float *B, int64_t ldb, int64_t strideB, float *C,
                        int64_t ldc, int batch, float *workspace, eap_stream_t stream);

int eap_gemm_bf16x3_f32_supported(int M, int N, int K, const float *A, int64_t lda, const float *B, int64_t ldb,
                                  int64_t strideB);
int eap_gemm_bf16x3_f32(int M, int N, int K, const float *A, int64_t lda, const float *B, int64_t ldb, int64_t strideB,
                        float *C, int64_t ldc, int64_t strideC, int batch, eap_stream_t stream);
int eap_gemm_bf16x3_presplit(int on);
int eap_gemm_bf16x3_nn_f32_supported(int M, int N, int K, const float *A, int64_t lda, const float *B, int64_t ldb,
                                     int64_t strideB);
int eap_gemm_bf16x3_nn_f32(int M, int N, int K, const float *A, int64_t lda, const float *B, int64_t ldb, int64_t strideB,
                           float *C, int64_t ldc, int64_t strideC, int batch, eap_stream_t stream);
int eap_gemm_bf16x3_ep_f32(int transB, int M, int N, int K, const float *A, int64_t lda, const float *B, int64_t ldb, int64_t strideB,
                           float *C, int64_t ldc, int64_t strideC, int batch, const float *scale, const float *shift, float slope,
                           const float *residual, int64_t strideRes, eap_stream_t stream);
int eap_gemm_bf16x3_reduce_f32_supported(int M, int N, int K, const float *A, int64_t lda, int64_t strideA, const float *B,
                                         int64_t ldb, int64_t strideB, int64_t ldc);
int64_t eap_gemm_bf16x3_reduce_workspace(int M, int N, int K, int batch);
int eap_gemm_bf16x3_reduce_f32(int M, int N, int K, const float *A, int64_t lda, int64_t strideA, const float *B, int64_t ldb,
                               int64_t strideB, float *C, int64_t ldc, int batch, float *workspace, eap_stream_t stream);
int eap_so3_intra_conv_bf16x3_f32_supported(int b, int o, int c, int p, int na, int nt);
int eap_so3_intra_conv_bf16x3_f32(int b, int o, int c, int p, int na, int nt, const float *W, const float *feats,
                                  const int32_t *intra_idx, float *out, eap_stream_t stream);
int eap_absmax_rows_f32(const float *x, int batch, int rows, int cols, int64_t ld, int64_t stride, int32_t *out_bits, eap_stream_t stream);
int eap_absmax_colgroups_f32(const float *x, int batch, int rows, int cols, int64_t ld, int64_t stride, int grp, int32_t *out_bits,
                             eap_stream_t stream);
int eap_so3_grouped_bound_f32(int b, int p, int nn, int n_sup, const int32_t *point_max_bits, const int32_t *idx, int32_t *out_bits,
                              eap_stream_t stream);
int eap_gemm_f16x2_f32(int trans_b, int M, int N, int K, const float *A, int64_t lda, const float *B, int64_t ldb, int64_t strideB,
                       float *C, int64_t ldc, int64_t strideC, int batch, const int32_t *abs_a, const int32_t *abs_b, int grp_b, float mult_b,
                       const float *scale, const float *shift, float slope, const float *residual, int64_t strideRes,
                       eap_stream_t stream);
int eap_gemm_f16x2_splitk_slabs(int M, int N, int K, int batch, int cus);
int64_t eap_gemm_f16x2_splitk_workspace(int M, int N, int batch, int slabs);
int eap_gemm_f16x2_splitk_f32(int M, int N, int K, const float *A, int64_t lda, const float *B, int64_t ldb, int64_t strideB,
                              float *C, int64_t ldc, int64_t strideC, int batch, const int32_t *abs_a, const int32_t *abs_b, int grp_b,
                              float mult_b, int slabs, float *workspace, int64_t workspace_floats, eap_stream_t stream);
int eap_so3_intra_conv_f16x2_f32(int b, int o, int c, int p, int na, int nt, const float *W, const float *feats,
                                 const int32_t *intra_idx, float *out, const int32_t *abs_w, const int32_t *abs_f, eap_stream_t stream);


int eap_gemm_dma_f32_supported(int transA, int transB, int M, int N, int K, const float *A, int64_t lda,
                               int64_t strideA, const float *B, int64_t ldb, int64_t strideB);
int eap_gemm_dma_f32(int transA, int transB, int M, int N, int K, const float *A, int64_t lda, int64_t strideA,
                     const float *B, int64_t ldb, int64_t strideB, float *C, int64_t ldc, int64_t strideC,
                     int batch, eap_stream_t stream);
int64_t eap_gemm_dma_f32_reduce_workspace(int M, int N, int K, int batch);
int eap_gemm_dma_f32_reduce(int transA, int transB, int M, int N, int K, const float *A, int64_t lda,
                            int64_t strideA, const float *B, int64_t ldb, int64_t strideB, float *C, int64_t ldc,
                            int batch, float *workspace, eap_stream_t stream);
int eap_gemm_skinny_reduce_f32_supported(int M, int N, int K, const float *A, int64_t lda, int64_t strideA, const float *B,
                                         int64_t ldb, int64_t strideB);
int64_t eap_gemm_skinny_reduce_workspace(int M, int N, int K, int batch);
int eap_gemm_skinny_reduce_f32(int M, int N, int K, const float *A, int64_t lda, int64_t strideA, const float *B, int64_t ldb,
                               int64_t strideB, float *C, int64_t ldc, int batch, float *workspace, eap_stream_t stream);

int eap_so3_inter_group_fwd_can_block(int c, int n, int na, int ks, int has_mult, int has_flag);
int eap_so3_inter_group_fwd_xb_f32(int b, int c, int p, int n, int nn, int na, int ks, float sigma,
                                   const float *feats, const int32_t *idx, const float *gx,
                                   const float *rk, const uint8_t *mult, const int32_t *nonident,
                                   float *out, eap_stream_t stream);
int eap_so3_inter_group_fwd_t_f32(int b, int c, int p, int n, int nn, int na, int ks, float sigma,
                                  const float *feats, const int32_t *idx, const float *gx,
                                  const float *rk, const uint8_t *mult, const int32_t *nonident,
                                  float *out, eap_stream_t stream);
int eap_gemm_f32_xb(int transA, int transB, int M, int N, int K, const float *A, int64_t lda,
                    int64_t strideA, const float *B, int64_t b_block_rows, int64_t strideB, float *C,
                    int64_t ldc, int64_t strideC, int batch, eap_stream_t stream);
int eap_gemm_f32_reduce_xb(int transA, int transB, int M, int N, int K, const float *A, int64_t lda,
                           int64_t strideA, const float *B, int64_t b_block_rows, int64_t strideB,
                           float *C, int64_t ldc, int batch, float *workspace, eap_stream_t stream);

int eap_so3_intra_conv_f32(int b, int o, int c, int p, int na, int nt, const float *W, const float *feats,
                           const int32_t *intra_idx, float *out, eap_stream_t stream);


int eap_so3_intra_group2d_fwd_f32(int b, int c, int p, int na, int nr, int t, const float *feats, const int32_t *intra_idx, float *out,
                                  eap_stream_t stream);
int eap_so3_intra_group2d_bwd_f32(int b, int c, int p, int na, int nr, int t, const float *gout, const int32_t *intra_idx, float *gfeats,
                                  eap_stream_t stream);
int eap_so3_intra_conv2d_f32(int b, int o, int c, int p, int na, int nr, int nt, const float *W, const float *feats,
                             const int32_t *intra_idx, float *out, eap_stream_t stream);
int eap_so3_intra_conv2d_split_supported(int b, int o, int c, int p, int na, int nr, int nt);
int eap_so3_intra_conv2d_bf16x3_f32(int b, int o, int c, int p, int na, int nr, int nt, const float *W, const float *feats,
                                    const int32_t *intra_idx, float *out, eap_stream_t stream);
int eap_so3_intra_conv2d_f16x2_f32(int b, int o, int c, int p, int na, int nr, int nt, const float *W, const float *feats,
                                   const int32_t *intra_idx, float *out, const int32_t *abs_w, const int32_t *abs_f, eap_stream_t stream);


int eap_chamfer_fwd_f32(int b, int n, int m, const float *xyz1, const float *xyz2, float *dist1,
                        float *dist2, int32_t *idx1, int32_t *idx2, eap_stream_t stream);
int eap_chamfer_fwd_f64(int b, int n, int m, const double *xyz1, const double *xyz2, double *dist1,
                        double *dist2, int32_t *idx1, int32_t *idx2, eap_stream_t stream);
int eap_chamfer_bwd_f32(int b, int n, int m, const float *xyz1, const float *xyz2,
                        const int32_t *idx1, const int32_t *idx2, const float *g1, const float *g2,
                        float *gxyz1, float *gxyz2, eap_stream_t stream);
int eap_chamfer_bwd_ordered_f32(int b, int n, int m, const float *xyz1, const float *xyz2,
                                const int32_t *idx1, const int32_t *idx2, const float *g1, const float *g2,
                                float *gxyz1, float *gxyz2, eap_stream_t stream);
int eap_chamfer_bwd_ordered_f64(int b, int n, int m, const double *xyz1, const double *xyz2,
                                const int32_t *idx1, const int32_t *idx2, const double *g1, const double *g2,
                                double *gxyz1, double *gxyz2, eap_stream_t stream);

int eap_bn_act_segments(int64_t n);
int eap_bn_stats_f32(int b, int c, int64_t n, const float *x, float *psum, float *psq, eap_stream_t stream);
int eap_bn_act_fwd_f32(int b, int c, int64_t n, float slope, const float *x, const float *scale,
                       const float *shift, float *y, eap_stream_t stream);
int eap_bn_act_add_fwd_f32(int b, int c, int64_t n, float slope, const float *x, const float *scale,
                           const float *shift, const float *res, float *y, eap_stream_t stream);
int eap_bn_act_bwd_reduce_f32(int b, int c, int64_t n, float slope, const float *gy, const float *x,
                              const float *scale, const float *shift, const float *mean,
                              const float *invstd, float *pg, float *pgx, eap_stream_t stream);
int eap_bn_act_bwd_apply_f32(int b, int c, int64_t n, float slope, const float *gy, const float *x,
                             const float *scale, const float *shift, const float *mean,
                             const float *invstd, const float *k2, const float *k3, float *gx,
                             eap_stream_t stream);
int eap_bn_act_bwd_apply_rowmax_f32(int b, int c, int64_t n, int na, float slope, const float *gy, const float *x,
                                    const float *scale, const float *shift, const float *mean, const float *invstd,
                                    const float *k2, const float *k3, float *gx, uint32_t *rowmax, eap_stream_t stream);
int eap_bn_act_fromy_blocks(int64_t n, int na);
int eap_bn_act_bwd_reduce_fromy_f32(int b, int c, int64_t n, int na, float slope, const float *gy, const float *y, const float *beta,
                                    const float *inv_gamma, float *pg, float *pgx, uint32_t *gmax, uint32_t *xmax, eap_stream_t stream);

int eap_bn_stats_masked_f32(int b, int c, int64_t n, int na, const float *x, const float *mask, float *psum, float *psq,
                            eap_stream_t stream);
int eap_bn_act_cloud_fwd_f32(int b, int c, int64_t n, float slope, const float *x, const float *scale, const float *shift,
                             float *y, eap_stream_t stream);
int eap_bn_act_cloud_bwd_reduce_f32(int b, int c, int64_t n, float slope, const float *gy, const float *x, const float *scale,
                                    const float *shift, const float *mean, const float *invstd, float *pg, float *pgx,
                                    eap_stream_t stream);
int eap_bn_act_cloud_bwd_apply_f32(int b, int c, int64_t n, int na, float slope, const float *gy, const float *x,
                                   const float *scale, const float *shift, const float *mean, const float *invstd,
                                   const float *k2, const float *k3, const float *mask, float *gx, eap_stream_t stream);

int eap_narrow_contract_supported(int b, int o, int c, int64_t n);
int eap_narrow_contract_fwd_f32(int b, int o, int c, int64_t n, const float *W, const float *x, float *y, eap_stream_t stream);
int eap_narrow_contract_dx_f32(int b, int o, int c, int64_t n, const float *W, const float *g, float *dx, eap_stream_t stream);
int eap_narrow_contract_dw_slabs(int64_t n);
int eap_narrow_contract_dw_f32(int b, int o, int c, int64_t n, const float *g, const float *x, float *partial, eap_stream_t stream);

int eap_narrow_conv_segments(int64_t n);
int eap_narrow_conv_stats_f32(int b, int o, int ck, int64_t n, const float *W, const float *x, float *pivot, float *psum, float *psq,
                              eap_stream_t stream);
int eap_narrow_conv_bnact_fwd_f32(int b, int o, int ck, int64_t n, float slope, const float *W, const float *x, const float *scale,
                                  const float *shift, float *y, eap_stream_t stream);
int eap_narrow_conv_bwd_reduce_f32(int b, int o, int ck, int64_t n, float slope, const float *gy, const float *x, const float *W,
                                   const float *scale, const float *shift, const float *mean, const float *invstd, float *pg, float *pgx,
                                   eap_stream_t stream);
int eap_narrow_conv_bwd_dw_f32(int b, int o, int ck, int64_t n, float slope, const float *gy, const float *x, const float *W,
                               const float *scale, const float *shift, const float *mean, const float *invstd, const float *k2,
                               const float *k3, float *partial, float *dW, eap_stream_t stream);

int eap_norm_fold_train_f32(int o, int parts, int64_t pivot_stride, int64_t count, int64_t eps_bits, int64_t momentum_bits, const float *ps,
                            const float *pq, const float *pivot, const float *gamma, const float *beta, float *running_mean, float *running_var,
                            float *scale, float *shift, double *mean, double *invstd, float *beta_copy, float *inv_gamma, eap_stream_t stream);
int eap_norm_fold_bwd_f32(int o, int parts, int b, int na, int64_t count, const float *pg, const float *pgx, const float *k1, const float *beta,
                          const float *inv_gamma, const float *gmax, const float *xmax, float *dgamma, float *dbeta, float *k2, float *k3, float *coef,
                          float *bound, float *colmax, eap_stream_t stream);
int eap_so3_dense_zbound_f32(int b, int na, int rp, int p, int ldz, int64_t cnt_stride, const float *colmax, const int32_t *cnt,
                             const int32_t *n_rows, float *words, eap_stream_t stream);
int eap_so3_dense_gplanes_bound_f32(int b, int o, int c, int na, int ks, int rp, const float *W3, const float *fc4, float *fpart, float *wsum,
                                    float *bound, eap_stream_t stream);
int eap_so3_dense_point_order(int b, int p, int words, const int64_t *order, const uint32_t *memb, const float *q_xyz, int32_t *order32,
                              uint32_t *memb_out, float *xyz_out, int32_t *pivot_pos, eap_stream_t stream);

int eap_anchor_attn_pool_fwd_f32(int b, int c, int n, int na, float temperature, const float *x, const float *logits,
                                 float *out, float *conf, eap_stream_t stream);
int eap_anchor_attn_pool_bwd_f32(int b, int c, int n, int na, float temperature, const float *x, const float *logits,
                                 const float *g, float *dx, float *dlogits, eap_stream_t stream);
int eap_slot_masked_mean_fwd_f32(int b, int ns, int c, int n, int na, const float *x, const float *mask,
                                 const float *inv_den, float *out, eap_stream_t stream);
int eap_slot_masked_mean_bwd_f32(int b, int ns, int c, int n, int na, const float *g, const float *mask,
                                 const float *inv_den, float *dx, eap_stream_t stream);
int eap_masked_max_fwd_f32(int b, int c, int n, int na, const float *x, const float *mask, float *out, int32_t *arg,
                           eap_stream_t stream);
int eap_masked_max_bwd_f32(int b, int c, int n, int na, const float *g, const int32_t *arg, const float *mask, float *dx,
                           eap_stream_t stream);
int eap_anchor_attn_pool_wide_fwd_f32(int b, int c, int n, int na, float temperature, const float *x, const float *logits,
                                      float *out, float *conf, eap_stream_t stream);
int eap_anchor_attn_pool_wide_bwd_f32(int b, int c, int n, int na, float temperature, const float *x, const float *logits,
                                      const float *g, float *dx, float *dlogits, eap_stream_t stream);
int eap_slot_masked_mean_wide_fwd_f32(int b, int ns, int c, int n, int na, const float *x, const float *mask,
                                      const float *inv_den, float *out, eap_stream_t stream);
int eap_slot_masked_mean_wide_bwd_f32(int b, int ns, int c, int n, int na, const float *g, const float *mask,
                                      const float *inv_den, float *dx, eap_stream_t stream);
int eap_masked_max_wide_fwd_f32(int b, int c, int n, int na, const float *x, const float *mask, float *out, int32_t *arg,
                                eap_stream_t stream);
int eap_masked_max_wide_bwd_f32(int b, int c, int n, int na, const float *g, const int32_t *arg, const float *mask, float *dx,
                                eap_stream_t stream);
int eap_bn_act_cloud_mean_fwd_f32(int b, int c, int n, int na, float slope, const float *x, const float *scale, const float *shift,
                                  const float *w, const float *inv_den, float *out, eap_stream_t stream);
int eap_bn_act_cloud_mean_parts(int n);
int eap_bn_act_cloud_mean_bwd_reduce_f32(int b, int c, int n, int na, float slope, const float *g, const float *x, const float *scale,
                                         const float *shift, const float *mean, const float *invstd, const float *w, const float *inv_den,
                                         float *pg, float *pgx, eap_stream_t stream);
int eap_bn_act_cloud_mean_bwd_apply_f32(int b, int c, int n, int na, float slope, const float *g, const float *x, const float *scale,
                                        const float *shift, const float *mean, const float *invstd, const float *k2, const float *k3,
                                        const float *w, const float *inv_den, const float *stat_mask, float *gx, eap_stream_t stream);
int eap_bn_act_cloud_mean_wide_fwd_f32(int b, int c, int n, int na, float slope, const float *x, const float *scale, const float *shift,
                                       const float *w, const float *inv_den, float *out, eap_stream_t stream);
int eap_bn_act_cloud_mean_wide_parts(int n);
int eap_bn_act_cloud_mean_wide_bwd_reduce_f32(int b, int c, int n, int na, float slope, const float *g, const float *x, const float *scale,
                                              const float *shift, const float *mean, const float *invstd, const float *w, const float *inv_den,
                                              float *pg, float *pgx, eap_stream_t stream);
int eap_bn_act_cloud_mean_wide_bwd_apply_f32(int b, int c, int n, int na, float slope, const float *g, const float *x, const float *scale,
                                             const float *shift, const float *mean, const float *invstd, const float *k2, const float *k3,
                                             const float *w, const float *inv_den, const float *stat_mask, float *gx, eap_stream_t stream);

int eap_slot_attn_stats_f32(int b, int d, int n, float ln_eps, const float *x, float *mean, float *rstd, eap_stream_t stream);
int eap_slot_attn_scores_fwd_f32(int b, int s, int d, int n, float eps, const float *x, const float *mean, const float *rstd, const float *u,
                                 const float *c0, float *attn, eap_stream_t stream);
int eap_slot_attn_pool_parts(int n);
int eap_slot_attn_pool_f32(int b, int s, int d, int n, const float *x, const float *mean, const float *rstd, const float *w, float *psum,
                           eap_stream_t stream);
int eap_slot_attn_scores_bwd_f32(int b, int s, int d, int n, float eps, const float *x, const float *mean, const float *rstd, const float *attn,
                                 const float *gmsum, const float *gwsum, const float *gattn, float *gdots, eap_stream_t stream);
int eap_slot_attn_input_grad_f32(int b, int j, int d, int n, const float *x, const float *mean, const float *rstd, const float *rows,
                                 const float *vecs, float *gx, eap_stream_t stream);

int eap_pointnet_max_parts(int n);
int eap_pointnet_max_fwd_f32(int b, int c, int o, int n, int na, const float *feats, const float *xyz, const float *centre, const float *member,
                             const float *wt, const float *v, const float *bias, float *pval, int32_t *parg, float *out, int32_t *arg,
                             eap_stream_t stream);
int eap_pointnet_max_bwd_data_f32(int b, int c, int o, int n, int na, const float *g, const int32_t *arg, const float *w, int ldw, float *dfeats,
                                  float *dcoords, eap_stream_t stream);
int eap_pointnet_max_bwd_weight_f32(int b, int c, int o, int n, int na, const float *g, const int32_t *arg, const float *feats, const float *xyz,
                                    const float *centre, const float *anchors, float *dwp, eap_stream_t stream);

#ifdef __cplusplus
}
#endif
#endif
```

Baseline: 171.2 point-clouds/sec.

## Consume compact row gradients in backward reductions instead of scattered dense gradients

The dense backward leaves a hint pairing the scattered gradient with its compact per-row form and row list. Downstream BN-activation reduce, narrow-conv reduce and the BN split kernels can then read the compact gradient through a point-to-slot map. Points with no referenced row are treated as zero gradient, so their gradient loads are skipped and only activation min/max bounds are kept. This cuts memory traffic on the sparse gradient, at the cost of a slot-map kernel, indirect loads and more code paths.

Result: no change. 171.8 point-clouds/sec, median of 4 (+0.3%).

```diff
diff --git a/equi-articulated-pose_amd/csrc/bn_act.hip b/equi-articulated-pose_amd/csrc/bn_act.hip
--- a/equi-articulated-pose_amd/csrc/bn_act.hip
+++ b/equi-articulated-pose_amd/csrc/bn_act.hip
@@ -202,10 +202,12 @@
     }
 }
 
+struct FromyRows { const int32_t *slot_of; int rp; };
+template <bool ROWS>
 __global__ __launch_bounds__(256) void bn_act_bwd_reduce_fromy_kernel(int c, long n4, int nq, int nblk, float slope, float inv_slope, const float4 *__restrict__ gy,
                                                                       const float4 *__restrict__ y, const float *__restrict__ beta,
                                                                       const float *__restrict__ inv_gamma, float *__restrict__ pg, float *__restrict__ pgx,
-                                                                      unsigned *__restrict__ gmax, unsigned *__restrict__ xmax) {
+                                                                      unsigned *__restrict__ gmax, unsigned *__restrict__ xmax, FromyRows rows) {
     __shared__ unsigned s_max[256][8];
     const int ci = blockIdx.y, bi = blockIdx.z, t = threadIdx.x;
     const int T = nq * (256 / nq);
@@ -216,16 +218,33 @@
     unsigned mg[4] = {0, 0, 0, 0}, mx[4] = {0, 0, 0, 0};
     if (t < T) {
         float4 g[RM_PIECES], a[RM_PIECES];
-#pragma unroll
-        for (int v = 0; v < RM_PIECES; ++v) {
-            const long i = base + (long)v * T + t;
-            if (i < n4) { g[v] = gy[r0 + i]; a[v] = y[r0 + i]; }
-        }
+        unsigned with_g = ROWS ? 0u : ~0u;
+        float ylo[4] = {INFINITY, INFINITY, INFINITY, INFINITY}, yhi[4] = {-INFINITY, -INFINITY, -INFINITY, -INFINITY};
 #pragma unroll
         for (int v = 0; v < RM_PIECES; ++v) {
             const long i = base + (long)v * T + t;
             if (i < n4) {
-                const float gv[4] = {g[v].x, g[v].y, g[v].z, g[v].w}, yv[4] = {a[v].x, a[v].y, a[v].z, a[v].w};
+                if constexpr (ROWS) {
+                    const long pt = ((long)blockIdx.x * RM_PIECES + v) * (T / nq) + t / nq;
+                    const int sl = rows.slot_of[(size_t)bi * (size_t)(n4 / nq) + pt];
+                    if (sl >= 0) { g[v] = gy[(((size_t)bi * c + ci) * rows.rp + sl) * nq + t % nq]; with_g |= 1u << v; }
+                } else {
+                    g[v] = gy[r0 + i];
+                }
+                a[v] = y[r0 + i];
+            }
+        }
+#pragma unroll
+        for (int v = 0; v < RM_PIECES; ++v) {
+            const long i = base + (long)v * T + t;
+            if (i < n4) {
+                const float yv[4] = {a[v].x, a[v].y, a[v].z, a[v].w};
+                if (ROWS && !((with_g >> v) & 1u)) {
+#pragma unroll
+                    for (int e = 0; e < 4; ++e) { ylo[e] = fminf(ylo[e], yv[e]); yhi[e] = fmaxf(yhi[e], yv[e]); }
+                    continue;
+                }
+                const float gv[4] = {g[v].x, g[v].y, g[v].z, g[v].w};
 #pragma unroll
                 for (int e = 0; e < 4; ++e) {
                     const bool pos = yv[e] > 0.f;
@@ -236,6 +255,14 @@
                     mx[e] = max(mx[e], __float_as_uint(xh) & 0x7fffffffu);
                 }
             }
+        }
+        if constexpr (ROWS) {
+#pragma unroll
+            for (int e = 0; e < 4; ++e)
+                if (ylo[e] <= yhi[e]) {
+                    const float xl = ((ylo[e] > 0.f ? ylo[e] : ylo[e] * inv_slope) - be) * ig, xu = ((yhi[e] > 0.f ? yhi[e] : yhi[e] * inv_slope) - be) * ig;
+                    mx[e] = max(mx[e], max(__float_as_uint(xl) & 0x7fffffffu, __float_as_uint(xu) & 0x7fffffffu));
+                }
         }
     }
 #pragma unroll
@@ -334,8 +361,26 @@
     if (int e = eap::hip_fail(hipMemsetAsync(gmax, 0, sizeof(uint32_t) * (size_t)b * c * na, s), "bn_act_bwd_reduce_fromy memset")) return e;
     if (int e = eap::hip_fail(hipMemsetAsync(xmax, 0, sizeof(uint32_t) * (size_t)b * c * na, s), "bn_act_bwd_reduce_fromy memset")) return e;
     const int nq = na / 4, nblk = eap_bn_act_fromy_blocks(n, na);
-    return eap::run_kernel("bn_act_bwd_reduce_fromy", bn_act_bwd_reduce_fromy_kernel, nblk, c, b, dim3(256), 0, s, c, (long)(n / 4), nq, nblk, slope,
-                           1.0f / slope, reinterpret_cast<const float4 *>(gy), reinterpret_cast<const float4 *>(y), beta, inv_gamma, pg, pgx, gmax, xmax);
+    return eap::run_kernel("bn_act_bwd_reduce_fromy", bn_act_bwd_reduce_fromy_kernel<false>, nblk, c, b, dim3(256), 0, s, c, (long)(n / 4), nq, nblk, slope,
+                           1.0f / slope, reinterpret_cast<const float4 *>(gy), reinterpret_cast<const float4 *>(y), beta, inv_gamma, pg, pgx, gmax, xmax,
+                           FromyRows{nullptr, 0});
+}
+
+extern "C" int eap_bn_act_bwd_reduce_fromy_rows_f32(int b, int c, int64_t n, int na, int rp, float slope, const float *gr, const int32_t *slot_of,
+                                                    const float *y, const float *beta, const float *inv_gamma, float *pg, float *pgx, uint32_t *gmax,
+                                                    uint32_t *xmax, eap_stream_t stream) {
+    if (int e = eap::rows_form_refuses("bn_act_bwd_reduce_fromy_rows", b, c, (long long)n, na, rp, gr, slot_of)) return e;
+    if (y == nullptr || beta == nullptr || inv_gamma == nullptr || pg == nullptr || pgx == nullptr || gmax == nullptr || xmax == nullptr)
+        return eap::bad_arg("bn_act_bwd_reduce_fromy_rows: null pointer");
+    if (na > 256 || n % na != 0 || !(slope > 0.f) || (reinterpret_cast<uintptr_t>(y) & 15) != 0)
+        return eap::bad_arg("bn_act_bwd_reduce_fromy_rows: rows of [points][na], na a multiple of 4 up to 256, 16-byte aligned tensors, a positive slope");
+    hipStream_t s = eap::S(stream);
+    if (int e = eap::hip_fail(hipMemsetAsync(gmax, 0, sizeof(uint32_t) * (size_t)b * c * na, s), "bn_act_bwd_reduce_fromy_rows memset")) return e;
+    if (int e = eap::hip_fail(hipMemsetAsync(xmax, 0, sizeof(uint32_t) * (size_t)b * c * na, s), "bn_act_bwd_reduce_fromy_rows memset")) return e;
+    const int nq = na / 4, nblk = eap_bn_act_fromy_blocks(n, na);
+    return eap::run_kernel("bn_act_bwd_reduce_fromy_rows", bn_act_bwd_reduce_fromy_kernel<true>, nblk, c, b, dim3(256), 0, s, c, (long)(n / 4), nq, nblk, slope,
+                           1.0f / slope, reinterpret_cast<const float4 *>(gr), reinterpret_cast<const float4 *>(y), beta, inv_gamma, pg, pgx, gmax, xmax,
+                           FromyRows{slot_of, rp});
 }
 
 namespace {
diff --git a/equi-articulated-pose_amd/csrc/common.h b/equi-articulated-pose_amd/csrc/common.h
--- a/equi-articulated-pose_amd/csrc/common.h
+++ b/equi-articulated-pose_amd/csrc/common.h
@@ -42,6 +42,19 @@
 
 template <typename... P>
 static inline bool aligned16(const P *...p) { return ((reinterpret_cast<uintptr_t>(p) | ... | (uintptr_t)0) & 15) == 0; }
+
+static inline int rows_form_refuses(const char *who, int b, int c, long long n, int na, int rp, const void *gr, const void *slot_of) {
+    char buf[200];
+    const char *why = nullptr;
+    if (b <= 0 || c <= 0 || n <= 0 || na <= 0 || rp <= 0) why = "positive sizes";
+    else if ((rp & 3) != 0 || (na & 3) != 0) why = "rp and na that are multiples of 4";
+    else if (gr == nullptr || slot_of == nullptr) why = "a compact gradient and a slot map (null pointer)";
+    else if ((reinterpret_cast<uintptr_t>(gr) & 15) != 0) why = "a 16-byte aligned compact gradient";
+    else if ((long long)b * c * rp * (na / 4) > 0x7fffffffLL) why = "a compact gradient of at most 2^31 16-byte pieces";
+    if (!why) return 0;
+    snprintf(buf, sizeof(buf), "%s: the row form takes %s", who, why);
+    return bad_arg(buf);
+}
 
 static inline int launch_dims(const char *what, long long gx, long long gy, long long gz, dim3 block, dim3 *grid) {
     const bool block_ok = block.x >= 1 && block.y >= 1 && block.z >= 1 && block.x <= 1024 && block.y <= 1024 && block.z <= 1024 &&
diff --git a/equi-articulated-pose_amd/csrc/inv_lists.hip b/equi-articulated-pose_amd/csrc/inv_lists.hip
--- a/equi-articulated-pose_amd/csrc/inv_lists.hip
+++ b/equi-articulated-pose_amd/csrc/inv_lists.hip
@@ -164,6 +164,14 @@
     if (q >= 0) dst[(((size_t)bi * c + ci) * n + q) * na4 + a] = src[(((size_t)bi * c + ci) * rcap + r) * na4 + a];
 }
 
+__global__ __launch_bounds__(256) void rows_slot_map_kernel(int n, int rp, int rld, const int32_t *__restrict__ rows,
+                                                            const int32_t *__restrict__ n_rows, int32_t *__restrict__ slot_of) {
+    const int bi = blockIdx.y, j = blockIdx.x * 256 + threadIdx.x;
+    if (j >= min(n_rows[bi], rp)) return;
+    const int r = rows[(size_t)bi * rld + j];
+    if ((unsigned)r < (unsigned)n) slot_of[(size_t)bi * n + r] = j;
+}
+
 }
 
 extern "C" int eap_inv_lists_rows(int b, int p, int n, int nn, const int32_t *idx, int32_t *counts, int32_t *rows,
@@ -211,3 +219,14 @@
     return eap::run_kernel("rows_scatter", rows_scatter_kernel, eap::cdiv((long long)rcap * (na / 4), 256), c, b, dim3(256), 0, s, c, n, na / 4, rcap, rows_ld, rows,
                            reinterpret_cast<const float4 *>(src), reinterpret_cast<float4 *>(dst));
 }
+
+extern "C" int eap_rows_slot_map_i32(int b, int n, int rp, int rows_ld, int n_rows_max, const int32_t *rows, const int32_t *n_rows,
+                                     int32_t *slot_of, eap_stream_t stream) {
+    if (b <= 0 || n <= 0 || rp <= 0 || rows_ld < rp) return eap::bad_arg("rows_slot_map: positive sizes, rows_ld >= rp");
+    if ((rp & 3) != 0) return eap::bad_arg("rows_slot_map: rp must be a multiple of 4");
+    if (n_rows_max < 0 || n_rows_max > rp) return eap::bad_arg("rows_slot_map: n_rows beyond rp");
+    if (rows == nullptr || n_rows == nullptr || slot_of == nullptr) return eap::bad_arg("rows_slot_map: null pointer");
+    hipStream_t s = eap::S(stream);
+    if (int e = eap::hip_fail(hipMemsetAsync(slot_of, 0xff, sizeof(int32_t) * (size_t)b * n, s), "rows_slot_map memset")) return e;
+    return eap::run_kernel("rows_slot_map", rows_slot_map_kernel, eap::cdiv(rp, 256), b, 1, dim3(256), 0, s, n, rp, rows_ld, rows, n_rows, slot_of);
+}
diff --git a/equi-articulated-pose_amd/csrc/narrow_conv.hip b/equi-articulated-pose_amd/csrc/narrow_conv.hip
--- a/equi-articulated-pose_amd/csrc/narrow_conv.hip
+++ b/equi-articulated-pose_amd/csrc/narrow_conv.hip
@@ -163,13 +163,20 @@
     }
 }
 
-template <int KS2>
+struct NarrowRows {
+    const int32_t *slot_of;
+    int rp, na, nq, npts;
+    unsigned magic;
+    __device__ __forceinline__ unsigned point_of(unsigned quad) const { return nq == 1 ? quad : __umulhi(quad, magic); }
+};
+
+template <int KS2, bool ROWS>
 __global__ __launch_bounds__(NT) void narrow_conv_bwd_reduce_kernel(int ct, int o, int ck, long n, int nseg, float slope,
                                                                       const float *__restrict__ gy, const float *__restrict__ x,
                                                                       const float *__restrict__ W, const float *__restrict__ scale,
                                                                       const float *__restrict__ shift, const float *__restrict__ mean,
                                                                       const float *__restrict__ invstd, float *__restrict__ pg,
-                                                                      float *__restrict__ pgx) {
+                                                                      float *__restrict__ pgx, NarrowRows rows) {
     __shared__ __attribute__((aligned(16))) float s_sc[64], s_sh[64], s_mu[64], s_is[64];
     __shared__ float s_red[WAVES][2][32];
     const Pos w(ct, n);
@@ -185,10 +192,21 @@
     const float *gb = gy + ((size_t)w.bi * o + w.ch0) * n;
     const unsigned roff = 4u * (4u * h * (unsigned)n + 4u * w.li);
     const int lc = w.ch0 - o0;
+    const size_t rpna = ROWS ? (size_t)rows.rp * rows.na : 0;
+    const float *grb = ROWS ? gy + ((size_t)w.bi * o + w.ch0 + 4 * h) * rpna : nullptr;
 #pragma unroll 1
     for (long col0 = w.beg + (long)w.cw * TILE; col0 < w.end; col0 += (long)w.ncw * TILE) {
         const long col = col0 + 4 * w.li;
         const bool ok = col < n;
+        const float *gl = nullptr;
+        if constexpr (ROWS) {
+            if (ok) {
+                const unsigned quad = (unsigned)(col >> 2), pt = rows.point_of(quad);
+                const int sl = pt < (unsigned)rows.npts ? rows.slot_of[(size_t)w.bi * rows.npts + pt] : -1;
+                if (sl >= 0) gl = grb + (size_t)sl * rows.na + 4u * (quad - pt * (unsigned)rows.nq);
+            }
+            if (__ballot(gl != nullptr) == 0) continue;
+        }
         f32x4 xa[KS2];
         load_x<KS2>(xa, xb, n, col0, w.xoff, ok, ck, h);
         f32x16 d[4];
@@ -198,7 +216,12 @@
             for (int g = 0; g < 4; ++g) {
                 f32x4 gv[4];
 #pragma unroll
-                for (int q = 0; q < 4; ++q) gv[q] = ld_off<f32x4>(gb + (size_t)(8 * g) * n + col0, roff + 4u * q * (unsigned)n);
+                for (int q = 0; q < 4; ++q) {
+                    if constexpr (ROWS)
+                        gv[q] = gl != nullptr ? *reinterpret_cast<const f32x4 *>(gl + (size_t)(8 * g + q) * rpna) : (f32x4){0.f, 0.f, 0.f, 0.f};
+                    else
+                        gv[q] = ld_off<f32x4>(gb + (size_t)(8 * g) * n + col0, roff + 4u * q * (unsigned)n);
+                }
                 const f32x4 sc = *reinterpret_cast<const f32x4 *>(&s_sc[lc + 8 * g + 4 * h]), sh = *reinterpret_cast<const f32x4 *>(&s_sh[lc + 8 * g + 4 * h]);
                 const f32x4 mu = *reinterpret_cast<const f32x4 *>(&s_mu[lc + 8 * g + 4 * h]), is = *reinterpret_cast<const f32x4 *>(&s_is[lc + 8 * g + 4 * h]);
 #pragma unroll
@@ -348,8 +371,33 @@
     if (b <= 0 || n <= 0) return 0;
     const int nseg = nseg_of((long)n), ct = tiles_per_block(o);
     return by_depth(ck, [&](auto ks2) {
-        return eap::run_kernel("narrow_conv_bwd_reduce", narrow_conv_bwd_reduce_kernel<decltype(ks2)::value>, nseg, o / (32 * ct), b, dim3(NT), 0, eap::S(stream),
-                               ct, o, ck, (long)n, nseg, slope, gy, x, W, scale, shift, mean, invstd, pg, pgx);
+        return eap::run_kernel("narrow_conv_bwd_reduce", narrow_conv_bwd_reduce_kernel<decltype(ks2)::value, false>, nseg, o / (32 * ct), b, dim3(NT), 0, eap::S(stream),
+                               ct, o, ck, (long)n, nseg, slope, gy, x, W, scale, shift, mean, invstd, pg, pgx, NarrowRows{});
+    });
+}
+
+namespace {
+inline int rows_view(const char *who, int b, int o, int ck, long n, int na, int rp, const float *gr, const int32_t *slot_of, const float *x, NarrowRows *rows) {
+    if (int e = eap::rows_form_refuses(who, b, o, n, na, rp, gr, slot_of)) return e;
+    if (n % na != 0) return eap::bad_arg("narrow_conv row form: n = points * na");
+    if (int e = refuse(who, o, ck, n, x, gr)) return e;
+    const int nq = na / 4;
+    *rows = NarrowRows{slot_of, rp, na, nq, (int)(n / na), nq > 1 ? (unsigned)(((1ull << 32) + nq - 1) / nq) : 0u};
+    return 0;
+}
+}
+
+extern "C" int eap_narrow_conv_bwd_reduce_rows_f32(int b, int o, int ck, int64_t n, int na, int rp, float slope, const float *gr, const int32_t *slot_of,
+                                                   const float *x, const float *W, const float *scale, const float *shift, const float *mean,
+                                                   const float *invstd, float *pg, float *pgx, eap_stream_t stream) {
+    NarrowRows rows;
+    if (int e = rows_view("narrow_conv_bwd_reduce_rows", b, o, ck, (long)n, na, rp, gr, slot_of, x, &rows)) return e;
+    if (x == nullptr || W == nullptr || scale == nullptr || shift == nullptr || mean == nullptr || invstd == nullptr || pg == nullptr || pgx == nullptr)
+        return eap::bad_arg("narrow_conv_bwd_reduce_rows: null pointer");
+    const int nseg = nseg_of((long)n), ct = tiles_per_block(o);
+    return by_depth(ck, [&](auto ks2) {
+        return eap::run_kernel("narrow_conv_bwd_reduce_rows", narrow_conv_bwd_reduce_kernel<decltype(ks2)::value, true>, nseg, o / (32 * ct), b, dim3(NT), 0,
+                               eap::S(stream), ct, o, ck, (long)n, nseg, slope, gr, x, W, scale, shift, mean, invstd, pg, pgx, rows);
     });
 }
 
diff --git a/equi-articulated-pose_amd/csrc/so3_dense.hip b/equi-articulated-pose_amd/csrc/so3_dense.hip
--- a/equi-articulated-pose_amd/csrc/so3_dense.hip
+++ b/equi-articulated-pose_amd/csrc/so3_dense.hip
@@ -280,11 +280,13 @@
 }
 
 struct SplitBn { const f32x4 *Y2; const float *coef; float slope, inv_slope; };
-template <bool BN>
+struct SplitRows { const int32_t *slot_of; int rp, l_src; };
+template <bool BN, bool ROWS = false>
 __global__ __launch_bounds__(256) __attribute__((amdgpu_waves_per_eu(2, 2))) void dense_split_kernel(int m, int l, int na, int kb_total, int seg, long long seg_pitch4, int mapped,
                                                           const int32_t *__restrict__ n_rows, const int32_t *__restrict__ colmap,
                                                           const f32x4 *__restrict__ T, const float *__restrict__ scale2,
-                                                          u32x4 *__restrict__ planes, SplitBn bn) {
+                                                          u32x4 *__restrict__ planes, SplitBn bn, SplitRows rows) {
+    static_assert(BN || !ROWS, "the rows form is the BatchNorm form's");
     extern __shared__ u32x4 image[];
     const int t = threadIdx.x;
     const int MT = m >> 5;
@@ -296,6 +298,7 @@
     if (mapped && n_rows != nullptr && 16 * kb >= ((min(n_rows[b], seg) + 15) & ~15) * nseg) return;
     const int l0 = 16 * kb + 8 * kg;
     unsigned at[8], keep[8];
+    int gat[ROWS ? 8 : 1];
     int live = 0;
     if (colmap != nullptr) {
         int ci[8] = {-1, -1, -1, -1, -1, -1, -1, -1};
@@ -305,6 +308,13 @@
         }
 #pragma unroll
         for (int e = 0; e < 8; ++e) { keep[e] = ci[e] >= 0 ? ~0u : 0u; at[e] = (unsigned)max(ci[e], 0) * (unsigned)nq; live |= (int)(keep[e] & 1u) << e; }
+        if constexpr (ROWS) {
+#pragma unroll
+            for (int e = 0; e < 8; ++e) {
+                const int sl = (ci[e] >= 0 && ci[e] < rows.l_src) ? rows.slot_of[(size_t)b * rows.l_src + ci[e]] : -1;
+                gat[e] = sl >= 0 ? sl * nq : -1;
+            }
+        }
     } else {
         int sg = l0 / seg, sr = l0 - sg * seg;
         if (mapped) dense_kr(l0, nseg, sg, sr);
@@ -317,6 +327,13 @@
         }
 #pragma unroll
         for (int e = 1; e < 8; ++e) at[e] = keep[e] ? at[e] : at[0];
+        if constexpr (ROWS) {
+#pragma unroll
+            for (int e = 0; e < 8; ++e) {
+                const int sl = l0 + e < min(l, rows.l_src) ? rows.slot_of[(size_t)b * rows.l_src + l0 + e] : -1;
+                gat[e] = sl >= 0 ? sl * nq : -1;
+            }
+        }
     }
     if (live == 0)
         for (int i = t; i < 64 * na; i += 256) image[i] = (u32x4){0u, 0u, 0u, 0u};
@@ -329,8 +346,14 @@
             const int row = 32 * mt + min(it0 + u * RG, 31);
             rowv[u] = row;
             const size_t row_off = ((size_t)b * m + row) * (colmap ? (size_t)1 : (size_t)nseg) * seg_pitch4 + aq;
-#pragma unroll
-            for (int e = 0; e < 8; ++e) q[u][e] = T[row_off + at[e]];
+            if constexpr (ROWS) {
+                const size_t g_off = ((size_t)b * m + row) * (size_t)rows.rp * nq + aq;
+#pragma unroll
+                for (int e = 0; e < 8; ++e) q[u][e] = gat[e] >= 0 ? T[g_off + gat[e]] : (f32x4){0.f, 0.f, 0.f, 0.f};
+            } else {
+#pragma unroll
+                for (int e = 0; e < 8; ++e) q[u][e] = T[row_off + at[e]];
+            }
             if constexpr (BN) {
 #pragma unroll
                 for (int e = 0; e < 8; ++e) q2[u][e] = bn.Y2[row_off + at[e]];
@@ -986,11 +1009,13 @@
                                         reinterpret_cast<const f32x4 *>(src), scale, scale2);
     if (e) return e;
     return eap::run_kernel("so3_dense_split", dense_split_kernel<false>, (long long)kb_total * (m / 32) * b * 2, 1, 1, dim3(256), (size_t)na * 1024, s, m, l, na, kb_total, seg, (long long)(seg_pitch / 4),
-                           mapped ? 1 : 0, n_rows, colmap, reinterpret_cast<const f32x4 *>(src), scale2, reinterpret_cast<u32x4 *>(planes), SplitBn{nullptr, nullptr, 1.f, 1.f});
-}
-
-extern "C" int eap_so3_dense_split_bn_f32(int b, int m, int l, int l_src, int na, const uint32_t *rowbound, const int32_t *colmap, const float *grad,
-                                          const float *act, const float *coef, float slope, float *scale, void *planes, eap_stream_t stream) {
+                           mapped ? 1 : 0, n_rows, colmap, reinterpret_cast<const f32x4 *>(src), scale2, reinterpret_cast<u32x4 *>(planes), SplitBn{nullptr, nullptr, 1.f, 1.f},
+                           SplitRows{nullptr, 0, 0});
+}
+
+namespace {
+int dense_split_bn(int b, int m, int l, int l_src, int na, const uint32_t *rowbound, const int32_t *colmap, const float *grad, const int32_t *slot_of,
+                   int rows_rp, const float *act, const float *coef, float slope, float *scale, void *planes, eap_stream_t stream) {
     if (b <= 0) return 0;
     if (colmap == nullptr && l != l_src) return eap::bad_arg("so3_dense_split_bn: without a column map l = l_src");
     if ((m % 32) != 0 || (na % 4) != 0 || na > 64 || ((reinterpret_cast<uintptr_t>(grad) | reinterpret_cast<uintptr_t>(act)) & 15) ||
@@ -1004,9 +1029,28 @@
                                 scale2))
         return e;
     const int seg = colmap ? l : l_src;
+    const SplitBn bn{reinterpret_cast<const f32x4 *>(act), coef, slope, 1.0f / slope};
+    if (rows_rp > 0)
+        return eap::run_kernel("so3_dense_split_bn_rows", dense_split_kernel<true, true>, (long long)kb_total * (m / 32) * b * 2, 1, 1, dim3(256), (size_t)na * 1024, s, m, l, na,
+                               kb_total, seg, (long long)l_src * na / 4, 0, nullptr, colmap, reinterpret_cast<const f32x4 *>(grad), scale2, reinterpret_cast<u32x4 *>(planes),
+                               bn, SplitRows{slot_of, rows_rp, l_src});
     return eap::run_kernel("so3_dense_split_bn", dense_split_kernel<true>, (long long)kb_total * (m / 32) * b * 2, 1, 1, dim3(256), (size_t)na * 1024, s, m, l, na, kb_total, seg,
-                           (long long)l_src * na / 4, 0, nullptr, colmap, reinterpret_cast<const f32x4 *>(grad), scale2, reinterpret_cast<u32x4 *>(planes),
-                           SplitBn{reinterpret_cast<const f32x4 *>(act), coef, slope, 1.0f / slope});
+                           (long long)l_src * na / 4, 0, nullptr, colmap, reinterpret_cast<const f32x4 *>(grad), scale2, reinterpret_cast<u32x4 *>(planes), bn,
+                           SplitRows{nullptr, 0, 0});
+}
+}
+
+extern "C" int eap_so3_dense_split_bn_f32(int b, int m, int l, int l_src, int na, const uint32_t *rowbound, const int32_t *colmap, const float *grad,
+                                          const float *act, const float *coef, float slope, float *scale, void *planes, eap_stream_t stream) {
+    return dense_split_bn(b, m, l, l_src, na, rowbound, colmap, grad, nullptr, 0, act, coef, slope, scale, planes, stream);
+}
+
+extern "C" int eap_so3_dense_split_bn_rows_f32(int b, int m, int l, int l_src, int na, int rp, const uint32_t *rowbound, const int32_t *colmap, const float *gr,
+                                               const int32_t *slot_of, const float *act, const float *coef, float slope, float *scale, void *planes,
+                                               eap_stream_t stream) {
+    if (int e = eap::rows_form_refuses("so3_dense_split_bn_rows", b, m, (long long)l_src, na, rp, gr, slot_of)) return e;
+    if (l <= 0 || act == nullptr || scale == nullptr || planes == nullptr) return eap::bad_arg("so3_dense_split_bn_rows: positive sizes, no null pointer");
+    return dense_split_bn(b, m, l, l_src, na, rowbound, colmap, gr, slot_of, rp, act, coef, slope, scale, planes, stream);
 }
 
 namespace {
diff --git a/equi-articulated-pose_amd/vgtk/_hip.py b/equi-articulated-pose_amd/vgtk/_hip.py
--- a/equi-articulated-pose_amd/vgtk/_hip.py
+++ b/equi-articulated-pose_amd/vgtk/_hip.py
@@ -1079,6 +1079,76 @@
     return rowmax
 
 
+_ROWS_HINT = [None]
+USE_ROWS_HINT = True
+ROWS_HINTS_TAKEN = 0
+
+
+class RowsGrad:
+
+    def __init__(self, gr, rows, n_rows, n):
+        b, c, rp, na = gr.shape
+        if not gr.is_contiguous() or gr.dtype != torch.float32 or rows.dtype != torch.int32 or n_rows.dtype != torch.int32 \
+                or rows.shape[0] != b or rows.shape[1] < rp or rows.stride(1) != 1 or tuple(n_rows.shape) != (b,):
+            raise RuntimeError('RowsGrad: gr float32 contiguous [b,c,rp,na], rows int32 [b,>=rp], n_rows int32 [b]')
+        self.gr, self.rows, self.n_rows, self.n, self.rp = gr, rows, n_rows, int(n), int(rp)
+        self._slot_of = None
+
+    @property
+    def slot_of(self):
+        if self._slot_of is None:
+            b = self.gr.shape[0]
+            self._slot_of = torch.empty(b, self.n, dtype=torch.int32, device=self.gr.device)
+            call('eap_rows_slot_map_i32', self.gr, b, self.n, self.rp, self.rows.stride(0), self.rp, self.rows, self.n_rows.contiguous(), self._slot_of)
+        return self._slot_of
+
+
+def leave_rows_hint(t, gr, rows, n_rows):
+    if USE_ROWS_HINT and gr.shape[2] % 4 == 0 and gr.shape[3] % 4 == 0 and gr.data_ptr() % 16 == 0:
+        _leave_hint(_ROWS_HINT, t, RowsGrad(gr, rows, n_rows, t.shape[2]))
+
+
+def take_rows_hint(t):
+    global ROWS_HINTS_TAKEN
+    h, _ROWS_HINT[0] = _ROWS_HINT[0], None
+    if not USE_ROWS_HINT or h is None or h[0]() is not t or h[1] != t._version or h[2] != tuple(t.shape):
+        return None
+    ROWS_HINTS_TAKEN += 1
+    return h[3]
+
+
+def bn_act_bwd_reduce_fromy_rows(rg, y, beta, inv_gamma, slope, partials=False):
+    b, c, p, na = y.shape
+    n = p * na
+    if tuple(rg.gr.shape[:2]) != (b, c) or rg.gr.shape[3] != na or rg.n != p:
+        raise RuntimeError('bn_act_bwd_reduce_fromy_rows: the compact gradient is not of this tensor')
+    check_input(y)
+    nblk = int(abi.eap_bn_act_fromy_blocks(n, na))
+    pg = torch.empty(c, b * nblk, dtype=torch.float32, device=y.device)
+    pgx = torch.empty_like(pg)
+    gmax = torch.empty(b, c, na, dtype=torch.int32, device=y.device)
+    xmax = torch.empty_like(gmax)
+    call('eap_bn_act_bwd_reduce_fromy_rows_f32', y, b, c, n, na, rg.rp, slope, rg.gr, rg.slot_of, y, beta, inv_gamma, pg, pgx, gmax, xmax)
+    if partials:
+        return pg, pgx, gmax.view(torch.float32), xmax.view(torch.float32)
+    return pg.sum(1, dtype=torch.float64), pgx.sum(1, dtype=torch.float64), gmax.view(torch.float32), xmax.view(torch.float32)
+
+
+def so3_dense_bwd_bn_rows(rg, yact, geo, ldz, coef, rowbound, slope):
+    b, o, p, na = yact.shape
+    if tuple(rg.gr.shape[:2]) != (b, o) or rg.gr.shape[3] != na or rg.n != p:
+        raise RuntimeError('so3_dense_bwd_bn_rows: the compact gradient is not of this tensor')
+    check_input(yact)
+    ldz = na * geo.rp if ldz is None else int(ldz)
+    colmap = geo.columns(None)
+    l = p if colmap is None else colmap.shape[1]
+    scale = torch.empty(2, b, na, o, dtype=torch.float32, device=yact.device)
+    planes = torch.empty(b * na * o * ((l + 31) // 32 * 32), dtype=torch.int32, device=yact.device)
+    call('eap_so3_dense_split_bn_rows_f32', yact, b, o, l, p, na, rg.rp, rowbound.view(torch.int32), colmap, rg.gr, rg.slot_of, yact, coef, slope, scale, planes)
+    z = torch.empty(b, o, geo.ks, ldz, dtype=torch.float32, device=yact.device)
+    return _dense_product(0, geo, b, o, l, ldz, scale, planes, z, 2.0 * b * o * l * na * geo.ks * geo.nn)
+
+
 def bn_act_bwd_apply(gy, x, b, c, n, scale, shift, mean, invstd, k2, k3, slope):
     gx = torch.empty_like(x)
     if x.dim() == 4 and x.shape[3] % 4 == 0 and x.shape[3] <= 64 and n == x.shape[2] * x.shape[3] and c % 128 == 0 and gx.data_ptr() % 16 == 0 \
@@ -1146,6 +1216,24 @@
     dW = torch.empty(o, ck, dtype=torch.float32, device=x.device)
     call('eap_narrow_conv_bwd_dw_f32', x, b, o, ck, n, slope, gy, x, W, scale, shift, mean, invstd, k2, k3, partial, dW)
     return dW
+
+
+def _narrow_rows_args(rg, x, W, na):
+    b, ck, n = x.shape
+    o = W.shape[0]
+    if tuple(rg.gr.shape[:2]) != (b, o) or rg.gr.shape[3] != na or rg.n * na != n:
+        raise RuntimeError('narrow_conv row form: the compact gradient is not of this layer\'s output')
+    return b, o, ck, n
+
+
+def narrow_conv_bwd_reduce_rows(rg, x, W, scale, shift, mean, invstd, slope, na, partials=False):
+    check_input(x, W, scale, shift, mean, invstd)
+    b, o, ck, n = _narrow_rows_args(rg, x, W, na)
+    pg, pgx = _narrow_partials(x, b, o, n)
+    call('eap_narrow_conv_bwd_reduce_rows_f32', x, b, o, ck, n, na, rg.rp, slope, rg.gr, rg.slot_of, x, W, scale, shift, mean, invstd, pg, pgx)
+    if partials:
+        return pg, pgx
+    return pg.sum(1, dtype=torch.float64), pgx.sum(1, dtype=torch.float64)
 
 
 
diff --git a/equi-articulated-pose_amd/vgtk/so3conv/functional.py b/equi-articulated-pose_amd/vgtk/so3conv/functional.py
--- a/equi-articulated-pose_amd/vgtk/so3conv/functional.py
+++ b/equi-articulated-pose_amd/vgtk/so3conv/functional.py
@@ -938,15 +938,24 @@
 def _backward_narrow(gy, W, x, bn, need_w):
     scale, shift, mean, invstd, count, slope, sync = bn
     b, o = gy.shape[0], gy.shape[1]
+    rg = _hip.take_rows_hint(gy) if (gy.dim() == 4 and gy.is_cuda) else None
+    if BACKWARD_LOG is not None and BACKWARD_LOG and BACKWARD_LOG[-1].get('regime') == 'narrow input':
+        BACKWARD_LOG[-1]['gradient'] = 'dense' if rg is None else 'rows'
+    na = gy.shape[3] if rg is not None else 0
     gy = gy.view(b, o, -1)
+    if rg is not None:
+        reduce_ = lambda **kw: _hip.narrow_conv_bwd_reduce_rows(rg, x, W, scale, shift, mean, invstd, slope, na, **kw)
+    else:
+        reduce_ = lambda **kw: _hip.narrow_conv_bwd_reduce(gy, x, W, scale, shift, mean, invstd, slope, **kw)
+    dw_ = lambda k2, k3: _hip.narrow_conv_bwd_dw(gy, x, W, scale, shift, mean, invstd, k2, k3, slope)
     if _native_norm_bwd(gy, count, sync):
-        g_bn_w, g_bn_b, k2, k3 = _hip.norm_fold_bwd(*_hip.narrow_conv_bwd_reduce(gy, x, W, scale, shift, mean, invstd, slope, partials=True), scale, count)
-        return (_hip.narrow_conv_bwd_dw(gy, x, W, scale, shift, mean, invstd, k2, k3, slope) if need_w else None), g_bn_w, g_bn_b
-    sg, sgx = _hip.narrow_conv_bwd_reduce(gy, x, W, scale, shift, mean, invstd, slope)
+        g_bn_w, g_bn_b, k2, k3 = _hip.norm_fold_bwd(*reduce_(partials=True), scale, count)
+        return (dw_(k2, k3) if need_w else None), g_bn_w, g_bn_b
+    sg, sgx = reduce_()
     gW = None
     if need_w:
         k2, k3 = norm_fold.backward_coefficients(scale, sg, sgx, count, True, sync)
-        gW = _hip.narrow_conv_bwd_dw(gy, x, W, scale, shift, mean, invstd, k2, k3, slope)
+        gW = dw_(k2, k3)
     return gW, sgx.float(), sg.float()
 
 
@@ -981,9 +990,10 @@
 def _backward_dense(gy, W, feats, head, geo, bn, yact, need_f, need_w):
     b, c, n, na = feats.shape
     o, ks, p, rp = W.shape[0], geo.ks, gy.shape[2], geo.rp
+    rg = _hip.take_rows_hint(gy) if (bn is not None and gy.is_cuda) else None
     if BACKWARD_LOG is not None:
         BACKWARD_LOG.append({'channels': (c, o), 'support_rows': n, 'referenced_rows_max': int(rp), 'regime': 'dense rows',
-                             **({'norm': 'in the node'} if bn is not None else {})})
+                             **({'norm': 'in the node', 'gradient': 'dense' if rg is None else 'rows'} if bn is not None else {})})
     ra = na * rp
     pad_c = 128 if (c == 64 and bn is not None) else c
     ldz = _hip.dense_pitch(ra) if (pad_c % 128 == 0 and (o * ks) % 16 == 0 and need_f) else ra
@@ -992,15 +1002,18 @@
         k1, beta, inv_gamma, count, slope, sync = bn
         native = _native_norm_bwd(gy, count, sync)
         if native:
-            pg, pgx, gmax, xmax = _hip.bn_act_bwd_reduce_fromy(gy, yact, beta, inv_gamma, slope, partials=True)
+            pg, pgx, gmax, xmax = (_hip.bn_act_bwd_reduce_fromy(gy, yact, beta, inv_gamma, slope, partials=True) if rg is None else
+                                   _hip.bn_act_bwd_reduce_fromy_rows(rg, yact, beta, inv_gamma, slope, partials=True))
             g_bn_w, g_bn_b, _, _, coef, bound, colmax = _hip.norm_fold_bwd(pg, pgx, k1, count, beta, inv_gamma, gmax, xmax)
         else:
-            sg, sgx, gmax, xmax = _hip.bn_act_bwd_reduce_fromy(gy, yact, beta, inv_gamma, slope)
+            sg, sgx, gmax, xmax = (_hip.bn_act_bwd_reduce_fromy(gy, yact, beta, inv_gamma, slope) if rg is None else
+                                   _hip.bn_act_bwd_reduce_fromy_rows(rg, yact, beta, inv_gamma, slope))
             g_bn_w, g_bn_b = sgx.float(), sg.float()
             k2, k3 = norm_fold.backward_coefficients(k1, sg, sgx, count, True, sync)
             coef = torch.stack([k1, k2, k3, beta, inv_gamma]).contiguous()
             bound = (k1.abs()[None, :, None] * gmax + k2.abs()[None, :, None] + k3.abs()[None, :, None] * xmax).contiguous()
-        z = _hip.so3_dense_bwd_bn(gy, yact, geo, ldz, coef, bound, slope)
+        z = (_hip.so3_dense_bwd_bn(gy, yact, geo, ldz, coef, bound, slope) if rg is None else
+             _hip.so3_dense_bwd_bn_rows(rg, yact, geo, ldz, coef, bound, slope))
         if ldz % 4 == 0 and rp % 4 == 0 and native:
             z_bound = (_hip.so3_dense_zbound(colmax, head.cnt, head.n_rows, rp, p, ldz).view(torch.int32), 4, 1.0)
         elif ldz % 4 == 0 and rp % 4 == 0:
@@ -1013,8 +1026,9 @@
     else:
         z = _hip.so3_dense_bwd(gy, geo, ldz)
     if need_f:
-        gFr = _rows_grad_from_z(z, _weight_operand(W, c, ks, pad_c), c, rp, na, ldz, True, z_bound)
-        gF = _hip.rows_scatter(gFr.contiguous(), head.rows, n)
+        gFr = _rows_grad_from_z(z, _weight_operand(W, c, ks, pad_c), c, rp, na, ldz, True, z_bound).contiguous()
+        gF = _hip.rows_scatter(gFr, head.rows, n)
+        _hip.leave_rows_hint(gF, gFr, head.rows, head.n_rows)
     if need_w:
         gW = _weight_grad_rows(z, _hip.rows_gather(feats, head.rows, rp), o, ks, ldz, True)
     return gF, gW, g_bn_w, g_bn_b
diff --git a/include/eap_hip.h b/include/eap_hip.h
--- a/include/eap_hip.h
+++ b/include/eap_hip.h
@@ -191,6 +191,8 @@
                         const float *src, float *dst, eap_stream_t stream);
 int eap_rows_scatter_f32(int b, int c, int n, int na, int rcap, int rows_ld, const int32_t *rows,
                          const float *src, float *dst, eap_stream_t stream);
+int eap_rows_slot_map_i32(int b, int n, int rp, int rows_ld, int n_rows_max, const int32_t *rows, const int32_t *n_rows,
+                          int32_t *slot_of, eap_stream_t stream);
 
 int eap_so3_dense_supported(int p, int na, int ks, int rp, int o);
 int eap_so3_dense_member(int b, int p, int n, int nn, int rp, int rows_ld, const int32_t *idx, const int32_t *rows,
@@ -212,6 +214,9 @@
                                             float *y, float *psum, float *psq, eap_stream_t stream);
 int eap_so3_dense_split_bn_f32(int b, int m, int l, int l_src, int na, const uint32_t *rowbound, const int32_t *colmap, const float *grad,
                                const float *act, const float *coef, float slope, float *scale, void *planes, eap_stream_t stream);
+int eap_so3_dense_split_bn_rows_f32(int b, int m, int l, int l_src, int na, int rp, const uint32_t *rowbound, const int32_t *colmap, const float *gr,
+                                    const int32_t *slot_of, const float *act, const float *coef, float slope, float *scale, void *planes,
+                                    eap_stream_t stream);
 int eap_so3_dense_untranspose_bnact_f32(int b, int o, int p, int na, int p_dst, const int32_t *map, const float *yt, const float *bn_scale,
                                         const float *bn_shift, float slope, float *y, eap_stream_t stream);
 int eap_so3_dense_gplanes_supported(int o, int c, int na, int ks, int rp);
@@ -373,6 +378,9 @@
 int eap_bn_act_fromy_blocks(int64_t n, int na);
 int eap_bn_act_bwd_reduce_fromy_f32(int b, int c, int64_t n, int na, float slope, const float *gy, const float *y, const float *beta,
                                     const float *inv_gamma, float *pg, float *pgx, uint32_t *gmax, uint32_t *xmax, eap_stream_t stream);
+int eap_bn_act_bwd_reduce_fromy_rows_f32(int b, int c, int64_t n, int na, int rp, float slope, const float *gr, const int32_t *slot_of,
+                                         const float *y, const float *beta, const float *inv_gamma, float *pg, float *pgx, uint32_t *gmax,
+                                         uint32_t *xmax, eap_stream_t stream);
 
 int eap_bn_stats_masked_f32(int b, int c, int64_t n, int na, const float *x, const float *mask, float *psum, float *psq,
                             eap_stream_t stream);
@@ -402,6 +410,9 @@
 int eap_narrow_conv_bwd_dw_f32(int b, int o, int ck, int64_t n, float slope, const float *gy, const float *x, const float *W,
                                const float *scale, const float *shift, const float *mean, const float *invstd, const float *k2,
                                const float *k3, float *partial, float *dW, eap_stream_t stream);
+int eap_narrow_conv_bwd_reduce_rows_f32(int b, int o, int ck, int64_t n, int na, int rp, float slope, const float *gr, const int32_t *slot_of,
+                                        const float *x, const float *W, const float *scale, const float *shift, const float *mean,
+                                        const float *invstd, float *pg, float *pgx, eap_stream_t stream);
 
 int eap_norm_fold_train_f32(int o, int parts, int64_t pivot_stride, int64_t count, int64_t eps_bits, int64_t momentum_bits, const float *ps,
                             const float *pq, const float *pivot, const float *gamma, const float *beta, float *running_mean, float *running_var,
```
